# wzf2000/GAMER

Measured on AMD Instinct MI355X. Metric: train-step sequences/sec, Qwen3Multi SMB decoder, his_len=100, higher is better.
Workload: dtype f32 tensors/accumulators, products = 3 x fp16 pieces (split3)

## Files before the change

### gamer_amd/_lib.py

```python
from __future__ import annotations

import ctypes as C
import os
import re
from typing import Optional

import torch

_HERE = os.path.dirname(os.path.abspath(__file__))
LIB_PATH = os.path.join(_HERE, "lib", "libgamer_hip.so")
if os.environ.get("GAMER_LIB_PATH"):
    LIB_PATH = os.path.abspath(os.environ["GAMER_LIB_PATH"])
HEADER_PATH = os.path.join(os.path.dirname(_HERE), "include", "gamer_hip.h")

_lib: Optional[C.CDLL] = None

c_void_p, c_int, c_float, c_int64, c_uint64 = C.c_void_p, C.c_int, C.c_float, C.c_int64, C.c_uint64


class GemmDesc(C.Structure):
    _fields_ = [
        ("A", c_void_p), ("a_rs", c_int64), ("a_ks", c_int64),
        ("B", c_void_p), ("b_rs", c_int64), ("b_ks", c_int64),
        ("C", c_void_p), ("ldc", c_int64),
        ("M", c_int), ("N", c_int), ("K", c_int),
        ("alpha", c_float),
        ("accumulate", c_int),
        ("groups", c_int),
        ("group_mode", c_int),
        ("group_offsets", c_void_p),
        ("strideB", c_int64), ("strideC", c_int64),
        ("kchunk", c_int),
        ("resid", c_void_p),
        ("row_map", c_void_p),
        ("p_drop", c_float),
        ("seed", c_uint64),
        ("rowdot_other", c_void_p),
        ("rowdot_out", c_void_p),
        ("rowdot_S", c_int),
        ("qk_wq", c_void_p), ("qk_wk", c_void_p),
        ("qk_eps", c_float),
        ("qk_cos", c_void_p), ("qk_sin", c_void_p),
        ("qk_bias_q", c_void_p), ("qk_bias_k", c_void_p), ("qk_bias_v", c_void_p),
        ("qk_act_idx", c_void_p),
        ("qk_pos_ids", c_void_p),
        ("qk_q_rot", c_void_p), ("qk_k_rot", c_void_p),
        ("qk_S", c_int), ("qk_nq", c_int), ("qk_nkv", c_int),
        ("b_planes", c_void_p), ("b_plane_stride", c_int64),
        ("amax_a", c_void_p), ("amax_b", c_void_p),
        ("amax_c", c_void_p), ("amax_c_col0", c_int),
        ("wgrad_ws", c_void_p), ("wgrad_ws_floats", c_int64),
        ("sw_gu", c_void_p), ("sw_ld", c_int64),
        ("group_div", c_int), ("sw_tbl", c_void_p), ("b_planes_t", c_void_p),
        ("sw_hm", c_void_p), ("sw_row_group", c_void_p),
    ]


class GemmBf16Desc(C.Structure):
    _fields_ = [
        ("A", c_void_p), ("lda", c_int64),
        ("B", c_void_p), ("ldb", c_int64),
        ("C", c_void_p), ("ldc", c_int64),
        ("M", c_int), ("N", c_int), ("K", c_int),
        ("accumulate", c_int),
        ("groups", c_int),
        ("group_mode", c_int),
        ("group_offsets", c_void_p),
        ("strideB", c_int64), ("strideC", c_int64),
        ("kchunk", c_int),
        ("resid", c_void_p),
        ("row_map", c_void_p),
        ("p_drop", c_float),
        ("seed", c_uint64),
        ("rowdot_other", c_void_p),
        ("rowdot_out", c_void_p),
        ("rowdot_S", c_int),
        ("qk_wq", c_void_p), ("qk_wk", c_void_p), ("qk_eps", c_float),
        ("qk_cos", c_void_p), ("qk_sin", c_void_p),
        ("qk_bias_q", c_void_p), ("qk_bias_k", c_void_p), ("qk_bias_v", c_void_p),
        ("qk_act_idx", c_void_p), ("qk_pos_ids", c_void_p),
        ("qk_q_rot", c_void_p), ("qk_k_rot", c_void_p),
        ("qk_S", c_int), ("qk_nq", c_int), ("qk_nkv", c_int),
        ("sw_gu", c_void_p), ("sw_ld", c_int64),
        ("wgrad_ws", c_void_p), ("wgrad_ws_floats", c_int64),
    ]


P, I, F, L, U = c_void_p, c_int, c_float, c_int64, c_uint64

_SIGNATURES = {
    "gamer_router_fwd": [P, P, P, P, I, I, I, I, I, I, P, P, P, P, P, P, P, P, P, P, P, P],
    "gamer_expert_lists": [P, I, I, I, P, P, P, P, P],
    "gamer_causal_prep": [P, I, I, P, P, P, P, P, P],
    "gamer_session_prep": [P, P, P, I, I, I, I, P, P, P, P, P, P, P],
    "gamer_moe_router_prep": [P, P, P, I, P, I, I, I, I, I, I, I, P, P, P, P, P, P, P, P, P],
    "gamer_embedding_fwd": [P, P, I, I, I, P, P],
    "gamer_embedding_bwd": [P, P, I, I, I, I, P, P],
    "gamer_embedding_bwd_ordered": [P, P, I, I, I, I, P, P, L, P],
    "gamer_embedding_bwd_ordered_ws_bytes": [I, I, I],
    "gamer_rmsnorm_fwd": [P, P, I, I, F, P, P, I, P],
    "gamer_rmsnorm_bwd": [P, P, P, I, P, I, I, F, I, P, P, I, P, P, F, U, P],
    "gamer_colsum_reduce": [P, I, I, I, P, P],
    "gamer_colsum_reduce_batched": [P, L, I, I, I, P, I, P],
    "gamer_rowtable_fwd": [P, P, P, I, I, P, I, I, P],
    "gamer_rowtable_bwd": [P, I, I, P, P, I, I, I, P, P, L, P],
    "gamer_gemm_f32": [C.POINTER(GemmDesc), P],
    "gamer_gemm_f32_split": [C.POINTER(GemmDesc), c_int, P],
    "gamer_split3_guard": [I],
    "gamer_gemm_bf16": [C.POINTER(GemmBf16Desc), P],
    "gamer_cast_params_bf16": [P, P, P, P, I, I, P],
    "gamer_attn_fwd_bf16": [P, I, P, I, P, I, P, P, I, I, I, I, F, F, U, P, P, P, P, P, P, P],
    "gamer_attn_bwd_bf16": [P, I, P, I, P, I, P, P, P, P, P, I, I, I, I, F, F, U, P, P, I, P, I, P, I, P, I, P, P, P, P],
    "gamer_session_spans": [P, P, P, P, P, I, I, I, I, P, P, P, P, P, P, P, P, P],
    "gamer_qknorm_rope_fwd": [P, I, I, I, I, P, P, F, P, P, P, P, P, P, P, P, P, P],
    "gamer_qknorm_rope_bwd": [P, P, P, I, I, I, I, P, P, F, P, P, P, P, P, I, P, P, P, P, P, P, P, P, L, P],
    "gamer_attn_row_order": [P, I, I, P, P, P, P],
    "gamer_attn_fwd": [P, I, P, I, P, I, P, P, P, P, I, I, I, I, F, F, U, P, P, P, P, P, I, P, P],
    "gamer_attn_bwd": [P, I, P, I, P, I, P, P, P, P, P, P, P, I, I, I, I, F, F, U, P, P, I, P, I, P, I, P, P, P, P, P, I, P],
    "gamer_split3_planes": [P, P, L, L, P],
    "gamer_absmax_f32": [P, I, L, I, I, L, P, P],
    "gamer_absmax_multi_f32": [P, P, I, P, P],
    "gamer_split2h_planes_multi": [P, P, I, P, P, P],
    "gamer_amax_sink": [P, P],
    "gamer_amax_sink3": [P, P, P],
    "gamer_attn_split_amax": [P, P, P, P],
    "gamer_attn_fwd_split": [P, I, P, I, P, I, P, P, P, I, I, I, I, F, F, U, P, P, P, P, P, I, P, P],
    "gamer_attn_bwd_split": [P, I, P, I, P, I, P, P, P, P, P, P, P, I, I, I, I, F, F, U, P, P, I, P, I, P, I, P, P, P, I, P, P, P],
    "gamer_residual_dropout_fwd": [P, P, P, I, I, F, U, P, P],
    "gamer_residual_dropout_bwd": [P, P, I, I, F, U, P, P],
    "gamer_swiglu_fwd": [P, P, L, F, U, P, P],
    "gamer_swiglu_bwd": [P, P, P, L, F, U, P],
    "gamer_swiglu_fwd_ld": [P, L, I, I, F, U, P, P],
    "gamer_swiglu_bwd_ld": [P, L, I, I, P, F, U, P],
    "gamer_swiglu_fwd_ld_tbl": [P, L, I, I, F, U, P, P, P, P],
    "gamer_swiglu_bwd_ld_tbl": [P, L, I, I, P, F, U, P, P, P],
    "gamer_silu_fwd_ld": [P, L, I, I, F, U, P, P],
    "gamer_silu_bwd_ld": [P, L, I, I, P, F, U, P],
# ... 113 lines not shown
```

### gamer_amd/csrc/common.h

```cpp
#pragma once
#include <hip/hip_runtime.h>
#include <stdint.h>
#include <stdio.h>
#include <stdarg.h>
#include <stdlib.h>

#include "../../include/gamer_hip.h"

namespace gamer {

void set_error(const char* fmt, ...);

#define GAMER_CHECK_ARG(cond, ...)                       \
    do {                                                 \
        if (!(cond)) {                                   \
            gamer::set_error(__VA_ARGS__);               \
            return -1;                                   \
        }                                                \
    } while (0)

#define GAMER_CHECK_LAUNCH(name)                                                        \
    do {                                                                                \
        hipError_t e__ = hipGetLastError();                                             \
        if (e__ != hipSuccess) {                                                        \
// ... 161 lines not shown
    __device__ __forceinline__ float mult(uint64_t idx) const {
        if (!on) return 1.f;
        uint32_t h = mix32((uint32_t)idx ^ k0);
        h = mix32(h + (uint32_t)(idx >> 32) * 0x9e3779b1U + k1);
        return h >= thr ? scale : 0.f;
    }
};

struct AttnDropout {
    uint32_t k0, k1, thr;
    float scale;
    __device__ __forceinline__ AttnDropout(float p, uint64_t seed) {
        k0 = mix32((uint32_t)seed ^ 0x9e3779b9U) ^ mix32((uint32_t)(seed >> 32) + 0x7f4a7c15U);
        k1 = mix32(k0 + 0x632be5abU);
        const float t = p * 4294967296.f;
        thr = t >= 4294967040.f ? 0xffffffffU : (uint32_t)t;
        scale = p > 0.f ? 1.f / (1.f - p) : 1.f;
    }
    __device__ __forceinline__ uint32_t row_word(uint32_t row) const {
        return (mix32(row * 0x9e3779b1U + k0) & 0xffffffU) | 0x800001U;
    }
    __device__ __forceinline__ uint32_t key_word(uint32_t j) const { return mix32(j * 0x85ebca6bU + k1) & 0xffffffU; }
    __device__ __forceinline__ bool keep(uint32_t a, uint32_t b) const { return __umul24(a, b) >= thr; }
};

__device__ __forceinline__ float xor32_max(float v) {
    const auto sw = __builtin_amdgcn_permlane32_swap(__float_as_uint(v), __float_as_uint(v), false, false);
    return fmaxf(__uint_as_float(sw[0]), __uint_as_float(sw[1]));
}
__device__ __forceinline__ float xor32_sum(float v) {
    const auto sw = __builtin_amdgcn_permlane32_swap(__float_as_uint(v), __float_as_uint(v), false, false);
    return __uint_as_float(sw[0]) + __uint_as_float(sw[1]);
}

__device__ __forceinline__ int wave_sum_i32(int v) {
#pragma unroll
    for (int o = 32; o > 0; o >>= 1) v += __shfl_xor(v, o, 64);
    return v;
}
__device__ __forceinline__ int wave_max_i32(int v) {
#pragma unroll
    for (int o = 32; o > 0; o >>= 1) v = max(v, __shfl_xor(v, o, 64));
    return v;
}
__device__ __forceinline__ int wave_min_i32(int v) {
#pragma unroll
    for (int o = 32; o > 0; o >>= 1) v = min(v, __shfl_xor(v, o, 64));
    return v;
}

#define GAMER_DPP_ROW_REDUCE(OP, v)                                                                   \
    v = OP(v, __builtin_amdgcn_update_dpp(v, v, 0xB1, 0xf, 0xf, false));      \
    v = OP(v, __builtin_amdgcn_update_dpp(v, v, 0x4E, 0xf, 0xf, false));      \
    v = OP(v, __builtin_amdgcn_update_dpp(v, v, 0x141, 0xf, 0xf, false));         \
    v = OP(v, __builtin_amdgcn_update_dpp(v, v, 0x140, 0xf, 0xf, false));
__device__ __forceinline__ int wave_min_i32_dpp(int v) {
    GAMER_DPP_ROW_REDUCE(min, v)
    return min(min(__builtin_amdgcn_readlane(v, 0), __builtin_amdgcn_readlane(v, 16)),
               min(__builtin_amdgcn_readlane(v, 32), __builtin_amdgcn_readlane(v, 48)));
}
__device__ __forceinline__ int wave_max_i32_dpp(int v) {
    GAMER_DPP_ROW_REDUCE(max, v)
    return max(max(__builtin_amdgcn_readlane(v, 0), __builtin_amdgcn_readlane(v, 16)),
               max(__builtin_amdgcn_readlane(v, 32), __builtin_amdgcn_readlane(v, 48)));
}

__device__ __forceinline__ float row16_sum_dpp(float v) {
#define GAMER_DPP_F(ctrl) __int_as_float(__builtin_amdgcn_update_dpp(__float_as_int(v), __float_as_int(v), ctrl, 0xf, 0xf, false))
    v += GAMER_DPP_F(0xB1);
    v += GAMER_DPP_F(0x4E);
    v += GAMER_DPP_F(0x141);
    v += GAMER_DPP_F(0x140);
#undef GAMER_DPP_F
    return v;
}

__device__ __forceinline__ float sigmoid_f(float x) { return __builtin_amdgcn_rcpf(1.f + __expf(-x)); }
__device__ __forceinline__ float silu_f(float x) { return x * sigmoid_f(x); }
__device__ __forceinline__ float dsilu_f(float x) {
    const float s = sigmoid_f(x);
    return s * (1.f + x * (1.f - s));
}

bool gemm_as_eligible(const gamer_gemm_desc* d, bool a_kc, bool b_kc, const uint16_t* b_planes);
int launch_gemm_as(const gamer_gemm_desc* d, const uint16_t* b_planes, bool b_kc, hipStream_t st);
bool gemm_os_eligible(const gamer_gemm_desc* d, bool a_kc, bool b_kc, const uint16_t* b_planes);
int launch_gemm_os(const gamer_gemm_desc* d, const uint16_t* b_planes, int guard, hipStream_t st, bool fwd_t = false);
bool gemm_os_fwd_eligible(const gamer_gemm_desc* d, bool a_kc, bool b_kc);
bool gemm_wg_eligible(const gamer_gemm_desc* d, bool a_kc, bool b_kc);
int launch_gemm_wg(const gamer_gemm_desc* d, hipStream_t st);

int launch_wgrad_reduce(const float* ws, float* C, int64_t ldc, int M, int N, int groups, const int32_t* group_offsets, int K,
                        int kchunk, int64_t strideC, hipStream_t st);

}
```

### gamer_amd/csrc/elementwise.hip

```cpp
#include "common.h"

namespace gamer {

constexpr int EW_THREADS = 256;
constexpr int EW_WAVES = EW_THREADS / WAVE;

#ifndef EW_MAX_BLOCKS_W
#define EW_MAX_BLOCKS_W 8192
#endif
#ifndef EW_MAX_BLOCKS_T
#define EW_MAX_BLOCKS_T 16384
#endif
static inline int grid_for_waves(int64_t n_waves, int max_blocks = EW_MAX_BLOCKS_W) {
    int64_t blocks = (n_waves + EW_WAVES - 1) / EW_WAVES;
    if (blocks < 1) blocks = 1;
    if (blocks > max_blocks) blocks = max_blocks;
    return (int)blocks;
}
static inline int grid_for_threads(int64_t n, int max_blocks = EW_MAX_BLOCKS_T) {
    int64_t blocks = (n + EW_THREADS - 1) / EW_THREADS;
    if (blocks < 1) blocks = 1;
    if (blocks > max_blocks) blocks = max_blocks;
    return (int)blocks;
}
// ... 149 lines not shown
            int rank = 0, cnt = 0;
            for (int j = 0; j < 64; ++j) {
                const int bj = __shfl(b, j, 64);
                const bool same = bj == b;
                rank += (same && j < lane) ? 1 : 0;
                cnt += same ? 1 : 0;
            }
            if (b >= 0) {
                const int pos = emb_cur[b] + rank;
                perm[pos] = t;
                __builtin_amdgcn_wave_barrier();
                if (rank == cnt - 1) emb_cur[b] = pos + 1;
            }
            __builtin_amdgcn_wave_barrier();
        }
    }
}

__global__ void __launch_bounds__(EW_THREADS)
emb_piece_sum_kernel(const float4* __restrict__ dx, int V, int H4, const int* __restrict__ row_start, const int* __restrict__ row_count,
                     const int* __restrict__ piece_start, const int* __restrict__ perm, float4* __restrict__ partial) {
    __shared__ float4 red[3][256];
    const int p = blockIdx.x;
    if (p >= piece_start[V]) return;
    int lo = 0, hi = V;
    while (hi - lo > 1) { const int mid = (lo + hi) >> 1; if (piece_start[mid] <= p) lo = mid; else hi = mid; }
    const int v = lo, k = p - piece_start[v];
    const int begin = row_start[v] + k * EMB_PIECE;
    const int count = min(EMB_PIECE, row_count[v] - k * EMB_PIECE);
    const int lane = threadIdx.x & 63, w = threadIdx.x >> 6;
    for (int c0 = 0; c0 < H4; c0 += 64) {
        const int c = c0 + lane;
        float4 acc = make_float4(0.f, 0.f, 0.f, 0.f);
        if (c < H4) {
            const int j1 = min(count, (w + 1) * (EMB_PIECE / 4));
            int j = w * (EMB_PIECE / 4);
            for (; j + 4 <= j1; j += 4) {
                const int r0 = perm[begin + j], r1 = perm[begin + j + 1], r2 = perm[begin + j + 2], r3 = perm[begin + j + 3];
                const float4 a0 = dx[(int64_t)r0 * H4 + c], a1 = dx[(int64_t)r1 * H4 + c], a2 = dx[(int64_t)r2 * H4 + c],
                             a3 = dx[(int64_t)r3 * H4 + c];
                acc.x = (((acc.x + a0.x) + a1.x) + a2.x) + a3.x; acc.y = (((acc.y + a0.y) + a1.y) + a2.y) + a3.y;
                acc.z = (((acc.z + a0.z) + a1.z) + a2.z) + a3.z; acc.w = (((acc.w + a0.w) + a1.w) + a2.w) + a3.w;
            }
            for (; j < j1; ++j) {
                const float4 a0 = dx[(int64_t)perm[begin + j] * H4 + c];
                acc.x += a0.x; acc.y += a0.y; acc.z += a0.z; acc.w += a0.w;
            }
        }
        if (w > 0 && c < H4) red[w - 1][lane] = acc;
        __syncthreads();
        if (w == 0 && c < H4) {
            const float4 b = red[0][lane], d = red[1][lane], e = red[2][lane];
            float4 o;
            o.x = (acc.x + b.x) + (d.x + e.x); o.y = (acc.y + b.y) + (d.y + e.y);
            o.z = (acc.z + b.z) + (d.z + e.z); o.w = (acc.w + b.w) + (d.w + e.w);
            partial[(int64_t)p * H4 + c] = o;
        }
        __syncthreads();
    }
}

__global__ void __launch_bounds__(64)
emb_row_sum_kernel(int H4, const int* __restrict__ piece_start, const float4* __restrict__ partial, float4* __restrict__ dW) {
    const int v = blockIdx.x;
    const int p0 = piece_start[v], p1 = piece_start[v + 1];
    if (p0 == p1) return;
    for (int c = threadIdx.x; c < H4; c += 64) {
        float4 s = partial[(int64_t)p0 * H4 + c];
        for (int p = p0 + 1; p < p1; ++p) {
            const float4 a = partial[(int64_t)p * H4 + c];
            s.x += a.x; s.y += a.y; s.z += a.z; s.w += a.w;
        }
        float4 o = dW[(int64_t)v * H4 + c];
        o.x += s.x; o.y += s.y; o.z += s.z; o.w += s.w;
        dW[(int64_t)v * H4 + c] = o;
    }
}

constexpr int RMS_MAXC_BIG = 4;

template <typename TY, int RMS_MAXC>
__global__ void __launch_bounds__(EW_THREADS)
rmsnorm_fwd_kernel(const float4* __restrict__ x, const float4* __restrict__ w, int T, int H4, float inv_h,
                   float eps, const int32_t* __restrict__ dst_rows, TY* __restrict__ y, int ldy, uint32_t* __restrict__ amax_out) {
    __shared__ uint32_t amax_lds[4];
    uint32_t am = 0;
    const int lane = threadIdx.x & 63;
    const int wave = (blockIdx.x * EW_THREADS + threadIdx.x) >> 6;
    const int nwaves = (gridDim.x * EW_THREADS) >> 6;
    float4 wv[RMS_MAXC];
#pragma unroll
    for (int i = 0; i < RMS_MAXC; ++i) {
        const int c = lane + 64 * i;
        wv[i] = (c < H4) ? w[c] : make_float4(0.f, 0.f, 0.f, 0.f);
    }
    for (int t = wave; t < T; t += nwaves) {
        float4 v[RMS_MAXC];
        float ss = 0.f;
#pragma unroll
        for (int i = 0; i < RMS_MAXC; ++i) {
            const int c = lane + 64 * i;
            v[i] = (c < H4) ? x[(int64_t)t * H4 + c] : make_float4(0.f, 0.f, 0.f, 0.f);
            ss += v[i].x * v[i].x + v[i].y * v[i].y + v[i].z * v[i].z + v[i].w * v[i].w;
        }
        ss = wave_sum(ss);
        const float rstd = rsqrtf(ss * inv_h + eps);
        const int64_t r = dst_rows ? dst_rows[t] : t;
        TY* yrow = y + r * ldy;
#pragma unroll
        for (int i = 0; i < RMS_MAXC; ++i) {
            const int c = lane + 64 * i;
            if (c < H4) {
                float4 o;
                o.x = wv[i].x * (v[i].x * rstd);
                o.y = wv[i].y * (v[i].y * rstd);
                o.z = wv[i].z * (v[i].z * rstd);
                o.w = wv[i].w * (v[i].w * rstd);
                st4(yrow + 4 * c, o);
                am = amax_f4(am, o);
            }
        }
    }
    amax_block_commit(am, amax_out, amax_lds);
}

template <typename TG, int RMS_MAXC>
__global__ void __launch_bounds__(EW_THREADS)
rmsnorm_bwd_kernel(const float4* __restrict__ x, const float4* __restrict__ w, const TG* __restrict__ dy,
                   int lddy, const int32_t* __restrict__ dy_rows, int T, int H4, float inv_h, float eps,
                   int accumulate_dx, float4* __restrict__ dx, float* __restrict__ dw_partial,
                   TG* __restrict__ mask_out, const int32_t* __restrict__ mask_rows, float p_drop, uint64_t seed,
                   uint32_t* __restrict__ amax_out) {
    const DropoutRng rng(mask_out ? p_drop : 0.f, seed);
    __shared__ float4 red[EW_WAVES][64 * RMS_MAXC];
    __shared__ uint32_t amax_lds[4];
    uint32_t am = 0;
    const int lane = threadIdx.x & 63;
    const int wib = threadIdx.x >> 6;
    const int wave = (blockIdx.x * EW_THREADS + threadIdx.x) >> 6;
    const int nwaves = (gridDim.x * EW_THREADS) >> 6;
    float4 wv[RMS_MAXC], dwacc[RMS_MAXC];
#pragma unroll
    for (int i = 0; i < RMS_MAXC; ++i) {
        const int c = lane + 64 * i;
        wv[i] = (c < H4) ? w[c] : make_float4(0.f, 0.f, 0.f, 0.f);
        dwacc[i] = make_float4(0.f, 0.f, 0.f, 0.f);
    }
    for (int t = wave; t < T; t += nwaves) {
        float4 v[RMS_MAXC], g[RMS_MAXC];
        float ss = 0.f;
        const int64_t r = dy_rows ? dy_rows[t] : t;
        const TG* dyrow = dy + r * lddy;
#pragma unroll
        for (int i = 0; i < RMS_MAXC; ++i) {
            const int c = lane + 64 * i;
            v[i] = (c < H4) ? x[(int64_t)t * H4 + c] : make_float4(0.f, 0.f, 0.f, 0.f);
            g[i] = (c < H4) ? ld4(dyrow + 4 * c) : make_float4(0.f, 0.f, 0.f, 0.f);
            ss += v[i].x * v[i].x + v[i].y * v[i].y + v[i].z * v[i].z + v[i].w * v[i].w;
        }
        ss = wave_sum(ss);
        const float rstd = rsqrtf(ss * inv_h + eps);
        float dot = 0.f;
#pragma unroll
        for (int i = 0; i < RMS_MAXC; ++i) {
            v[i].x *= rstd; v[i].y *= rstd; v[i].z *= rstd; v[i].w *= rstd;
            dwacc[i].x += g[i].x * v[i].x; dwacc[i].y += g[i].y * v[i].y;
            dwacc[i].z += g[i].z * v[i].z; dwacc[i].w += g[i].w * v[i].w;
            g[i].x *= wv[i].x; g[i].y *= wv[i].y; g[i].z *= wv[i].z; g[i].w *= wv[i].w;
            dot += g[i].x * v[i].x + g[i].y * v[i].y + g[i].z * v[i].z + g[i].w * v[i].w;
        }
        dot = wave_sum(dot) * inv_h;
#pragma unroll
        for (int i = 0; i < RMS_MAXC; ++i) {
            const int c = lane + 64 * i;
            if (c < H4) {
                float4 o;
                o.x = rstd * (g[i].x - v[i].x * dot);
                o.y = rstd * (g[i].y - v[i].y * dot);
                o.z = rstd * (g[i].z - v[i].z * dot);
                o.w = rstd * (g[i].w - v[i].w * dot);
                if (accumulate_dx) {
                    float4 p = dx[(int64_t)t * H4 + c];
                    o.x += p.x; o.y += p.y; o.z += p.z; o.w += p.w;
                }
                dx[(int64_t)t * H4 + c] = o;
                if (mask_out) {
                    float m[4];
                    rng.mult4((uint32_t)((int64_t)t * H4 + c), m);
                    const int64_t mr = mask_rows ? mask_rows[t] : t;
                    const float4 mo = make_float4(m[0] * o.x, m[1] * o.y, m[2] * o.z, m[3] * o.w);
                    st4(mask_out + (mr * H4 + c) * 4, mo);
                    am = amax_f4(am, mo);
                }
            }
        }
    }
#pragma unroll
    for (int i = 0; i < RMS_MAXC; ++i) red[wib][lane + 64 * i] = dwacc[i];
    __syncthreads();
    if (wib == 0) {
// ... 1366 lines not shown
extern "C" int gamer_amax_sink(uint32_t* out0, uint32_t* out1) {
    g_amax_sink.out[0] = out0;
    g_amax_sink.out[1] = out1;
    g_amax_sink.out[2] = nullptr;
    return 0;
}
extern "C" int gamer_amax_sink3(uint32_t* out0, uint32_t* out1, uint32_t* out2) {
    g_amax_sink.out[0] = out0;
    g_amax_sink.out[1] = out1;
    g_amax_sink.out[2] = out2;
    return 0;
}

extern "C" int gamer_embedding_fwd(const int64_t* ids, const float* W, int V, int T, int H, float* x, void* stream) {
    GAMER_CHECK_ARG(ids && W && x, "gamer_embedding_fwd: null pointer");
    GAMER_CHECK_ARG(T > 0 && H > 0 && H % 4 == 0 && V > 0, "gamer_embedding_fwd: bad shape T=%d H=%d V=%d", T, H, V);
    GAMER_CHECK_ARG(aligned16(W) && aligned16(x), "gamer_embedding_fwd: pointers must be 16-byte aligned");
    hipLaunchKernelGGL(embedding_fwd_kernel, dim3(grid_for_waves(T)), dim3(EW_THREADS), 0, ST(stream),
                       ids, (const float4*)W, V, T, H / 4, (float4*)x);
    GAMER_CHECK_LAUNCH("gamer_embedding_fwd");
    return 0;
}

extern "C" int gamer_embedding_bwd(const int64_t* ids, const float* dx, int V, int T, int H, int pad_id, float* dW,
                                   void* stream) {
    GAMER_CHECK_ARG(ids && dx && dW, "gamer_embedding_bwd: null pointer");
    GAMER_CHECK_ARG(T > 0 && H > 0 && V > 0, "gamer_embedding_bwd: bad shape T=%d H=%d V=%d", T, H, V);
    GAMER_CHECK_ARG(H <= 1024, "gamer_embedding_bwd: H=%d > 1024 unsupported", H);
    int chunk = EMB_CHUNK;
    while (chunk > 128 && (T + chunk - 1) / chunk < 512) chunk >>= 1;
    hipLaunchKernelGGL(embedding_bwd_kernel, dim3((T + chunk - 1) / chunk), dim3(EW_THREADS),
                       (size_t)EMB_CACHE * H * sizeof(float), ST(stream), ids, dx, V, T, H, pad_id, dW, chunk);
    GAMER_CHECK_LAUNCH("gamer_embedding_bwd");
    return 0;
}

extern "C" int64_t gamer_embedding_bwd_ordered_ws_bytes(int V, int T, int H) {
    if (V <= 0 || T <= 0 || H <= 0) return -1;
    const int64_t chunks = (T + EMB_SORT_CHUNK - 1) / EMB_SORT_CHUNK;
    const int64_t pieces = (int64_t)T / EMB_PIECE + V + 1;
    const int64_t ints = chunks * (V + 1) + 2 * (int64_t)(V + 1) + (V + 2) + T;
    return ((ints * 4 + 15) / 16) * 16 + pieces * H * 4;
}
extern "C" int gamer_embedding_bwd_ordered(const int64_t* ids, const float* dx, int V, int T, int H, int pad_id, float* dW,
                                           void* ws, int64_t ws_bytes, void* stream) {
    GAMER_CHECK_ARG(ids && dx && dW && ws, "gamer_embedding_bwd_ordered: null pointer");
    GAMER_CHECK_ARG(T > 0 && H > 0 && H % 4 == 0 && V > 0 && V <= EMB_MAX_V,
                    "gamer_embedding_bwd_ordered: bad shape T=%d H=%d V=%d (H %% 4 == 0, V <= %d)", T, H, V, EMB_MAX_V);
    GAMER_CHECK_ARG(aligned16(dx) && aligned16(dW) && aligned16(ws) && ws_bytes >= gamer_embedding_bwd_ordered_ws_bytes(V, T, H),
                    "gamer_embedding_bwd_ordered: dx / dW / ws must be 16-byte aligned and ws hold %lld bytes (got %lld)",
                    (long long)gamer_embedding_bwd_ordered_ws_bytes(V, T, H), (long long)ws_bytes);
    const int chunks = (T + EMB_SORT_CHUNK - 1) / EMB_SORT_CHUNK;
    const int pieces_max = T / EMB_PIECE + V + 1;
    int* ip = (int*)ws;
    EmbSortWs w;
    w.hist = ip; ip += (int64_t)chunks * (V + 1);
    w.row_start = ip; ip += V + 1;
    w.row_count = ip; ip += V + 1;
    w.piece_start = ip; ip += V + 2;
    w.perm = ip; ip += T;
    const int64_t ints = (int64_t)chunks * (V + 1) + 2 * (int64_t)(V + 1) + (V + 2) + T;
    w.partial = (float*)((char*)ws + ((ints * 4 + 15) / 16) * 16);
    hipStream_t st = ST(stream);
    const size_t lds = (size_t)(V + 1) * sizeof(int);
    hipLaunchKernelGGL(emb_hist_kernel, dim3(chunks), dim3(EW_THREADS), lds, st, ids, V, T, pad_id, w.hist);
    GAMER_CHECK_LAUNCH("gamer_embedding_bwd_ordered/hist");
    hipLaunchKernelGGL(emb_chunk_scan_kernel, dim3(V + 1), dim3(64), 0, st, V, chunks, w.hist, w.row_count);
    GAMER_CHECK_LAUNCH("gamer_embedding_bwd_ordered/chunk_scan");
    hipLaunchKernelGGL(emb_row_scan_kernel, dim3(1), dim3(1024), 0, st, V, w.row_count, w.row_start, w.piece_start);
    GAMER_CHECK_LAUNCH("gamer_embedding_bwd_ordered/row_scan");
    hipLaunchKernelGGL(emb_scatter_kernel, dim3(chunks), dim3(EW_THREADS), lds + EMB_SORT_CHUNK * sizeof(int), st, ids, V, T, pad_id,
                       w.hist, w.row_start, w.perm);
    GAMER_CHECK_LAUNCH("gamer_embedding_bwd_ordered/scatter");
    hipLaunchKernelGGL(emb_piece_sum_kernel, dim3(pieces_max), dim3(EW_THREADS), 0, st, (const float4*)dx, V, H / 4, w.row_start,
                       w.row_count, w.piece_start, w.perm, (float4*)w.partial);
    GAMER_CHECK_LAUNCH("gamer_embedding_bwd_ordered/pieces");
    hipLaunchKernelGGL(emb_row_sum_kernel, dim3(V), dim3(64), 0, st, H / 4, w.piece_start, (const float4*)w.partial, (float4*)dW);
    GAMER_CHECK_LAUNCH("gamer_embedding_bwd_ordered/rows");
    return 0;
}

template <typename TY>
static int rmsnorm_fwd_impl(const char* name, const float* x, const float* w, int T, int H, float eps,
                            const int32_t* dst_rows, TY* y, int ldy, void* stream) {
    GAMER_CHECK_ARG(x && w && y, "%s: null pointer", name);
    GAMER_CHECK_ARG(T > 0 && H > 0 && H % 4 == 0 && H <= 256 * RMS_MAXC_BIG && ldy >= H && ldy % 4 == 0,
                    "%s: bad shape T=%d H=%d ldy=%d (H%%4==0, H<=1024, ldy%%4==0)", name, T, H, ldy);
    GAMER_CHECK_ARG(aligned16(x) && aligned16(w) && aligned_vec4<TY>(y), "%s: pointers must be 16-byte aligned", name);
    const AmaxSink sink = take_amax_sink();
    if (H <= 256)
        hipLaunchKernelGGL((rmsnorm_fwd_kernel<TY, 1>), dim3(grid_for_waves(T)), dim3(EW_THREADS), 0, ST(stream),
                           (const float4*)x, (const float4*)w, T, H / 4, 1.f / (float)H, eps, dst_rows, y, ldy, sink.out[0]);
    else
        hipLaunchKernelGGL((rmsnorm_fwd_kernel<TY, RMS_MAXC_BIG>), dim3(grid_for_waves(T)), dim3(EW_THREADS), 0, ST(stream),
                           (const float4*)x, (const float4*)w, T, H / 4, 1.f / (float)H, eps, dst_rows, y, ldy, sink.out[0]);
    GAMER_CHECK_LAUNCH(name);
    return 0;
}
extern "C" int gamer_rmsnorm_fwd(const float* x, const float* w, int T, int H, float eps, const int32_t* dst_rows,
                                 float* y, int ldy, void* stream) {
    return rmsnorm_fwd_impl<float>("gamer_rmsnorm_fwd", x, w, T, H, eps, dst_rows, y, ldy, stream);
}
extern "C" int gamer_rmsnorm_fwd_bf16(const float* x, const float* w, int T, int H, float eps, const int32_t* dst_rows,
                                      gamer_bf16* y, int ldy, void* stream) {
    return rmsnorm_fwd_impl<bf16_t>("gamer_rmsnorm_fwd_bf16", x, w, T, H, eps, dst_rows, (bf16_t*)y, ldy, stream);
}

template <typename TG>
static int rmsnorm_bwd_impl(const char* name, const float* x, const float* w, const TG* dy, int lddy,
                            const int32_t* dy_rows, int T, int H, float eps, int accumulate_dx, float* dx,
                            float* dw_partial, int n_partial, TG* mask_out, const int32_t* mask_rows, float p_drop,
                            uint64_t seed, void* stream) {
    GAMER_CHECK_ARG(x && w && dy && dx && dw_partial, "%s: null pointer", name);
    GAMER_CHECK_ARG(T > 0 && H > 0 && H % 4 == 0 && H <= 256 * RMS_MAXC_BIG && lddy >= H && lddy % 4 == 0 && n_partial > 0,
                    "%s: bad shape T=%d H=%d lddy=%d n_partial=%d", name, T, H, lddy, n_partial);
    GAMER_CHECK_ARG(aligned16(x) && aligned16(w) && aligned_vec4<TG>(dy) && aligned16(dx) && aligned16(dw_partial) &&
                    aligned_vec4<TG>(mask_out), "%s: pointers must be 16-byte aligned", name);
    const AmaxSink sink = take_amax_sink();
    if (H <= 256)
        hipLaunchKernelGGL((rmsnorm_bwd_kernel<TG, 1>), dim3(n_partial), dim3(EW_THREADS), 0, ST(stream),
                           (const float4*)x, (const float4*)w, dy, lddy, dy_rows, T, H / 4, 1.f / (float)H, eps,
                           accumulate_dx, (float4*)dx, dw_partial, mask_out, mask_rows, p_drop, seed, sink.out[0]);
    else
        hipLaunchKernelGGL((rmsnorm_bwd_kernel<TG, RMS_MAXC_BIG>), dim3(n_partial), dim3(EW_THREADS), 0, ST(stream),
                           (const float4*)x, (const float4*)w, dy, lddy, dy_rows, T, H / 4, 1.f / (float)H, eps,
                           accumulate_dx, (float4*)dx, dw_partial, mask_out, mask_rows, p_drop, seed, sink.out[0]);
    GAMER_CHECK_LAUNCH(name);
    return 0;
}
extern "C" int gamer_rmsnorm_bwd(const float* x, const float* w, const float* dy, int lddy, const int32_t* dy_rows,
                                 int T, int H, float eps, int accumulate_dx, float* dx, float* dw_partial,
                                 int n_partial, float* mask_out, const int32_t* mask_rows, float p_drop,
                                 uint64_t seed, void* stream) {
    return rmsnorm_bwd_impl<float>("gamer_rmsnorm_bwd", x, w, dy, lddy, dy_rows, T, H, eps, accumulate_dx, dx, dw_partial,
                                   n_partial, mask_out, mask_rows, p_drop, seed, stream);
}
extern "C" int gamer_rmsnorm_bwd_bf16(const float* x, const float* w, const gamer_bf16* dy, int lddy,
                                      const int32_t* dy_rows, int T, int H, float eps, int accumulate_dx, float* dx,
                                      float* dw_partial, int n_partial, gamer_bf16* mask_out, const int32_t* mask_rows,
                                      float p_drop, uint64_t seed, void* stream) {
    return rmsnorm_bwd_impl<bf16_t>("gamer_rmsnorm_bwd_bf16", x, w, (const bf16_t*)dy, lddy, dy_rows, T, H, eps,
                                    accumulate_dx, dx, dw_partial, n_partial, (bf16_t*)mask_out, mask_rows, p_drop, seed,
                                    stream);
}

extern "C" int gamer_colsum_reduce(const float* partial, int rows, int cols, int accumulate, float* out, void* stream) {
    GAMER_CHECK_ARG(partial && out && rows > 0 && cols > 0, "gamer_colsum_reduce: bad arguments");
    hipLaunchKernelGGL(colsum_reduce_kernel, dim3((cols + 31) / 32), dim3(32 * COLSUM_RG), 0, ST(stream), partial, rows,
                       cols, accumulate, out);
    GAMER_CHECK_LAUNCH("gamer_colsum_reduce");
    return 0;
}

extern "C" int gamer_colsum_reduce_batched(const float* partial, int64_t stride, int rows, int cols, int n, float* const* outs,
                                           int accumulate, void* stream) {
    GAMER_CHECK_ARG(partial && outs && rows > 0 && cols > 0 && n > 0 && n <= 65535 && stride >= (int64_t)rows * cols,
                    "gamer_colsum_reduce_batched: bad arguments (rows=%d cols=%d n=%d stride=%lld)", rows, cols, n, (long long)stride);
    hipLaunchKernelGGL(colsum_reduce_batched_kernel, dim3((cols + 31) / 32, n), dim3(32 * COLSUM_RG), 0, ST(stream), partial, stride,
                       rows, cols, accumulate, outs);
    GAMER_CHECK_LAUNCH("gamer_colsum_reduce_batched");
    return 0;
}

template <typename TY>
static int rowtable_fwd_impl(const char* name, const float* table, const int32_t* idx, const int32_t* dst_rows, int T,
                             int E, TY* y, int ldy, int col0, void* stream) {
    GAMER_CHECK_ARG(table && idx && y, "%s: null pointer", name);
    GAMER_CHECK_ARG(T > 0 && E > 0 && E % 4 == 0 && ldy % 4 == 0 && col0 % 4 == 0 && col0 + E <= ldy,
                    "%s: bad shape T=%d E=%d ldy=%d col0=%d", name, T, E, ldy, col0);
    hipLaunchKernelGGL(rowtable_fwd_kernel<TY>, dim3(grid_for_threads((int64_t)T * E / 4)), dim3(EW_THREADS), 0,
                       ST(stream), (const float4*)table, idx, dst_rows, T, E / 4, y, ldy, col0, take_amax_sink().out[0]);
    GAMER_CHECK_LAUNCH(name);
    return 0;
}
extern "C" int gamer_rowtable_fwd(const float* table, const int32_t* idx, const int32_t* dst_rows, int T, int E,
                                  float* y, int ldy, int col0, void* stream) {
    return rowtable_fwd_impl<float>("gamer_rowtable_fwd", table, idx, dst_rows, T, E, y, ldy, col0, stream);
}
extern "C" int gamer_rowtable_fwd_bf16(const float* table, const int32_t* idx, const int32_t* dst_rows, int T, int E,
                                       gamer_bf16* y, int ldy, int col0, void* stream) {
    return rowtable_fwd_impl<bf16_t>("gamer_rowtable_fwd_bf16", table, idx, dst_rows, T, E, (bf16_t*)y, ldy, col0, stream);
}

template <typename TG>
// ... 496 lines not shown
```

### gamer_amd/csrc/gemm.hip

```cpp
#include "common.h"
#include <stdlib.h>

namespace gamer {

constexpr int BM = 128, BN = 128, BK = 32;
constexpr int GEMM_THREADS = 256;
constexpr int KC_LD = BK + 4;
constexpr int TILE_FLOATS = BM * KC_LD;
constexpr int GEMM_LDS_BYTES = 4 * TILE_FLOATS * (int)sizeof(float);

typedef float f32x16 __attribute__((ext_vector_type(16)));

constexpr int SP_KC_ROW = 80;
constexpr int SP_KC_IMG = BM * SP_KC_ROW;
constexpr int SP_RC_IMG = BK * 256;
constexpr int SP_OPERAND = 3 * SP_KC_IMG;
constexpr int SP_LDS_BYTES = 2 * SP_OPERAND;

#ifndef SP_ABLATE
#define SP_ABLATE 0
#endif
__device__ __forceinline__ uint32_t pack_hi16(uint32_t w0, uint32_t w1) { return __builtin_amdgcn_perm(w1, w0, 0x07060302u); }
__device__ __forceinline__ void split3(float x, uint32_t (&w)[3]) {
    if (SP_ABLATE & 1) { w[0] = w[1] = w[2] = __float_as_uint(x); return; }
// ... 1295 lines not shown
static int gemm_entry(const gamer_gemm_desc* d, void* stream, int split) {
    GAMER_CHECK_ARG(d, "gamer_gemm_f32: null descriptor");
    GAMER_CHECK_ARG(d->A && d->B && d->C, "gamer_gemm_f32: null matrix pointer");
    GAMER_CHECK_ARG(d->M > 0 && d->N > 0 && d->K > 0, "gamer_gemm_f32: bad shape M=%d N=%d K=%d", d->M, d->N, d->K);
    GAMER_CHECK_ARG((d->a_rs == 1) != (d->a_ks == 1) || (d->a_rs == 1 && d->a_ks == 1 && (d->M == 1 || d->K == 1)),
                    "gamer_gemm_f32: exactly one of a_rs/a_ks must be 1 (rs=%lld ks=%lld)", (long long)d->a_rs, (long long)d->a_ks);
    GAMER_CHECK_ARG((d->b_rs == 1) != (d->b_ks == 1) || (d->b_rs == 1 && d->b_ks == 1 && (d->N == 1 || d->K == 1)),
                    "gamer_gemm_f32: exactly one of b_rs/b_ks must be 1 (rs=%lld ks=%lld)", (long long)d->b_rs, (long long)d->b_ks);
    const bool a_kc = d->a_ks == 1, b_kc = d->b_ks == 1;
    const int64_t a_ld = a_kc ? d->a_rs : d->a_ks, b_ld = b_kc ? d->b_rs : d->b_ks;
    GAMER_CHECK_ARG(a_ld % 4 == 0 && b_ld % 4 == 0 && d->ldc >= d->N,
                    "gamer_gemm_f32: leading dims must be multiples of 4 (lda=%lld ldb=%lld ldc=%lld)",
                    (long long)a_ld, (long long)b_ld, (long long)d->ldc);
    GAMER_CHECK_ARG(aligned16(d->A) && aligned16(d->B), "gamer_gemm_f32: A and B must be 16-byte aligned");
    GAMER_CHECK_ARG(d->groups >= 1 && (d->groups == 1 || d->group_offsets), "gamer_gemm_f32: groups=%d needs group_offsets", d->groups);
    GAMER_CHECK_ARG(d->strideB % 4 == 0, "gamer_gemm_f32: strideB must be a multiple of 4");
    GAMER_CHECK_ARG(d->group_mode == 0 || d->group_mode == 1, "gamer_gemm_f32: group_mode=%d", d->group_mode);

    GemmParams p;
    p.A = d->A; p.a_rs = d->a_rs; p.a_ks = d->a_ks;
    p.B = d->B; p.b_rs = d->b_rs; p.b_ks = d->b_ks;
    p.C = d->C; p.ldc = d->ldc;
    p.M = d->M; p.N = d->N; p.K = d->K;
    p.alpha = d->alpha; p.accumulate = d->accumulate;
    p.groups = d->groups; p.group_offsets = d->group_offsets;
    p.strideB = d->strideB; p.strideC = d->strideC;
    p.kchunk = d->kchunk;
    p.resid = d->resid; p.row_map = d->row_map; p.p_drop = d->p_drop; p.seed = d->seed;
    p.rowdot_other = d->rowdot_other; p.rowdot_out = d->rowdot_out; p.rowdot_S = d->rowdot_S;
    p.qk_wq = d->qk_wq; p.qk_wk = d->qk_wk; p.qk_eps = d->qk_eps; p.qk_cos = d->qk_cos; p.qk_sin = d->qk_sin;
    p.qk_bias_q = d->qk_bias_q; p.qk_bias_k = d->qk_bias_k; p.qk_bias_v = d->qk_bias_v;
    p.qk_act_idx = d->qk_act_idx; p.qk_pos_ids = d->qk_pos_ids; p.qk_q_rot = d->qk_q_rot; p.qk_k_rot = d->qk_k_rot;
    p.qk_S = d->qk_S; p.qk_nq = d->qk_nq; p.qk_nkv = d->qk_nkv;
    p.amax_a = d->amax_a; p.amax_b = d->amax_b;
    p.guard = g_split3_guard;
    p.amax_c = d->amax_c; p.amax_c_col0 = d->amax_c_col0;
    p.wgrad_ws = nullptr;
    p.sw_gu = d->sw_gu; p.sw_ld = d->sw_ld;
    p.group_div = d->group_div > 1 ? d->group_div : 1; p.sw_tbl = d->sw_tbl;
    GAMER_CHECK_ARG(d->group_div <= 1 || (d->group_mode == 0 && d->group_offsets && d->groups % d->group_div == 0),
                    "gamer_gemm_f32: group_div = %d needs group_mode 0, group_offsets and groups (%d) a multiple of it", d->group_div, d->groups);
    GAMER_CHECK_ARG(!d->sw_tbl || ((d->sw_gu || d->sw_hm) && aligned16(d->sw_tbl)),
                    "gamer_gemm_f32: sw_tbl is an option of the SwiGLU epilogues (sw_gu, sw_hm)");
    GAMER_CHECK_ARG(!d->sw_gu || (split == 3 && d->group_mode == 0 && !d->accumulate && !d->resid && !d->rowdot_out && !d->qk_q_rot &&
                                  d->alpha == 1.f && d->N % 4 == 0 && d->sw_ld >= 2 * (int64_t)d->N && d->sw_ld % 4 == 0 &&
                                  aligned16(d->sw_gu) && d->p_drop >= 0.f && d->p_drop < 1.f),
                    "gamer_gemm_f32: the SwiGLU-backward epilogue (sw_gu) is built for gamer_gemm_f32_split(terms = 3), a plain input-"
                    "gradient GEMM with alpha = 1, N %% 4 == 0, sw_ld >= 2 N (N=%d sw_ld=%lld)", d->N, (long long)d->sw_ld);
    GAMER_CHECK_ARG(!d->amax_c || (d->group_mode == 0 && !d->accumulate && !d->resid && !d->qk_q_rot && d->amax_c_col0 >= 0 &&
                                   d->amax_c_col0 % 64 == 0),
                    "gamer_gemm_f32: amax_c needs a plain or row-dot Linear-forward / input-gradient GEMM (no accumulate, residual or "
                    "q|k|v epilogue) and amax_c_col0 a multiple of 64 (amax_c_col0=%d)", d->amax_c_col0);
    GAMER_CHECK_ARG(split != 3 || (d->amax_a && d->amax_b), "gamer_gemm_f32_split: terms = 3 needs amax_a and amax_b (gamer_absmax_f32)");
    p.b_planes = (split && d->group_mode == 0) ? (const uint16_t*)d->b_planes : nullptr;
    p.b_plane_stride = d->b_plane_stride;
    GAMER_CHECK_ARG(!p.b_planes || split == 3 || ((reinterpret_cast<uintptr_t>(p.b_planes) & 7u) == 0 && d->b_plane_stride % 4 == 0 && d->b_plane_stride > 0),
                    "gamer_gemm_f32_split: b_planes must be 8-byte aligned with b_plane_stride %% 4 == 0");
    GAMER_CHECK_ARG(!p.b_planes || split != 3 || (reinterpret_cast<uintptr_t>(p.b_planes) & 15u) == 0,
                    "gamer_gemm_f32_split: terms = 3 takes b_planes as packed pieces at B's offsets (16-byte aligned)");
    if (split == 3 && p.b_planes && ((b_kc ? d->K : d->N) % 4) != 0) p.b_planes = nullptr;
    GAMER_CHECK_ARG(!d->qk_q_rot || (d->qk_k_rot && d->qk_wq && d->qk_wk && d->qk_cos && d->qk_sin && d->group_mode == 0 &&
                                     d->groups == 1 && a_kc && b_kc && !d->resid && !d->rowdot_out && !d->accumulate &&
                                     d->alpha == 1.f && d->M % BM == 0 && d->qk_nq > 0 && d->qk_nkv > 0 && d->qk_S > 0 &&
                                     d->N == (d->qk_nq + 2 * d->qk_nkv) * 64 && d->N % BN == 0 && d->ldc % 4 == 0 &&
                                     aligned16(d->C) && aligned16(d->qk_q_rot) && aligned16(d->qk_k_rot) &&
                                     (!d->qk_bias_q || (d->qk_bias_k && d->qk_bias_v && d->qk_act_idx)) &&
                                     !diag_build_switches()),
                    "gamer_gemm_f32: the q|k|v epilogue needs a Linear-forward layout, one group, M %% 128 == 0 (M=%d), "
                    "N = (nq + 2 nkv) * 64 a multiple of 128 (N=%d), alpha = 1 and no other epilogue", d->M, d->N);
    GAMER_CHECK_ARG(!d->rowdot_out || (d->rowdot_other && d->rowdot_S > 0 && d->group_mode == 0 && d->groups == 1 &&
                                       !d->resid && !d->accumulate && d->M % BM == 0 && d->N % BN == 0 &&
                                       d->M % d->rowdot_S == 0 && d->ldc % 4 == 0 && aligned16(d->rowdot_other) &&
                                       aligned16(d->C) && !diag_build_switches()),
                    "gamer_gemm_f32: the row-dot epilogue needs full 128 x 128 tiles (M=%d N=%d), one group, ldc %% 4 == 0",
                    d->M, d->N);
    GAMER_CHECK_ARG(!d->resid || (d->group_mode == 0 && !d->accumulate && a_kc && b_kc && d->ldc % 4 == 0 &&
                                  aligned16(d->resid) && aligned16(d->C) && d->p_drop >= 0.f && d->p_drop < 1.f),
                    "gamer_gemm_f32: the fused residual epilogue needs a Linear-forward layout, ldc %% 4 == 0, no accumulate");
    GAMER_CHECK_ARG(!d->sw_hm || (d->group_mode == 0 && a_kc && b_kc && !d->accumulate && !d->resid && !d->rowdot_out && !d->qk_q_rot &&
                                  !d->sw_gu && d->alpha == 1.f && d->N % 8 == 0 && d->ldc >= d->N && d->ldc % 4 == 0 && aligned16(d->sw_hm) &&
                                  aligned16(d->C) && (!d->sw_tbl || d->sw_row_group) && d->p_drop >= 0.f && d->p_drop < 1.f),
                    "gamer_gemm_f32: the SwiGLU-forward epilogue (sw_hm) needs a Linear-forward layout with N = 2 I (N=%d), alpha = 1, no other "
                    "epilogue, and sw_row_group with sw_tbl", d->N);
    if (split == 3 && gemm_as_eligible(d, a_kc, b_kc, p.b_planes)) return launch_gemm_as(d, p.b_planes, b_kc, (hipStream_t)stream);
    if (d->sw_hm) {
        gamer_gemm_desc d2 = *d;
        d2.sw_hm = nullptr; d2.sw_row_group = nullptr; d2.sw_tbl = nullptr; d2.amax_c = nullptr;
        const int rc = gemm_entry(&d2, stream, split);
        if (rc) return rc;
        if (d->amax_c) gamer_amax_sink(d->amax_c, nullptr);
        return d->sw_tbl ? gamer_swiglu_fwd_ld_tbl(d->C, d->ldc, d->M, d->N / 2, d->p_drop, d->seed, d->sw_hm, d->sw_tbl, d->sw_row_group, stream)
                         : gamer_swiglu_fwd_ld(d->C, d->ldc, d->M, d->N / 2, d->p_drop, d->seed, d->sw_hm, stream);
    }
    if (split == 3 && gemm_os_eligible(d, a_kc, b_kc, p.b_planes)) return launch_gemm_os(d, p.b_planes, g_split3_guard, (hipStream_t)stream);
    if (split == 3 && gemm_os_fwd_eligible(d, a_kc, b_kc))
        return launch_gemm_os(d, reinterpret_cast<const uint16_t*>(d->b_planes_t), g_split3_guard, (hipStream_t)stream, true);
    p.n_tiles = (d->N + BN - 1) / BN;
    hipStream_t st = (hipStream_t)stream;

    if (d->group_mode == 0) {
        p.m_tiles = (d->M + BM - 1) / BM + (d->group_offsets ? d->groups : 0);
        const int64_t blocks = (int64_t)p.m_tiles * p.n_tiles;
        GAMER_CHECK_ARG(blocks < (1LL << 31), "gamer_gemm_f32: grid too large");
        if (a_kc && b_kc) return launch_gemm<true, true, 0>(p, (int)blocks, st, split);
        if (a_kc && !b_kc) return launch_gemm<true, false, 0>(p, (int)blocks, st, split);
        if (!a_kc && !b_kc) return launch_gemm<false, false, 0>(p, (int)blocks, st, split);
        GAMER_CHECK_ARG(false, "gamer_gemm_f32: layout (A row-contiguous, B k-contiguous) is not built");
    } else {
        GAMER_CHECK_ARG(!a_kc && !b_kc, "gamer_gemm_f32: group_mode 1 (wgrad) needs row-contiguous A and B");
        GAMER_CHECK_ARG(d->kchunk >= BK && d->kchunk % BK == 0, "gamer_gemm_f32: kchunk=%d must be a positive multiple of 32", d->kchunk);
        p.m_tiles = (d->M + BM - 1) / BM;
        const int64_t chunks = (d->K + d->kchunk - 1) / d->kchunk + (d->group_offsets ? d->groups : 0);
        const int64_t blocks = chunks * p.m_tiles * p.n_tiles;
        GAMER_CHECK_ARG(blocks < (1LL << 31), "gamer_gemm_f32: grid too large");
        p.wgrad_ws = d->wgrad_ws;
        if (p.wgrad_ws) {
            const int64_t need = chunks * p.m_tiles * p.n_tiles * (int64_t)(BM * BN);
            GAMER_CHECK_ARG(d->wgrad_ws_floats >= need && aligned16(d->wgrad_ws),
                            "gamer_gemm_f32: wgrad_ws holds %lld floats, this weight gradient needs %lld (chunks x tiles x 16384)",
                            (long long)d->wgrad_ws_floats, (long long)need);
            GAMER_CHECK_ARG(!diag_pp_switch(), "gamer_gemm_f32: the deterministic weight gradient is not built for the ping-pong form");
        }
        const int rc = (split == 3 && p.wgrad_ws && gemm_wg_eligible(d, a_kc, b_kc)) ? launch_gemm_wg(d, st)
                                                                                     : launch_gemm<false, false, 1>(p, (int)blocks, st, split);
        if (rc || !p.wgrad_ws) return rc;
        const int64_t rblocks = (int64_t)d->groups * p.m_tiles * p.n_tiles * 16;
        hipLaunchKernelGGL(wgrad_reduce_kernel, dim3((int)rblocks), dim3(256), 0, st, p.wgrad_ws, d->C, d->ldc, d->M, d->N, p.m_tiles,
                           p.n_tiles, d->groups, d->group_offsets, d->K, d->kchunk, d->strideC);
        GAMER_CHECK_LAUNCH("gamer_gemm_f32/wgrad_reduce");
        return 0;
    }
    return 0;
}

__device__ __forceinline__ uint32_t amax4(uint32_t m, const uint4 v) {
    return max(max(m, v.x & 0x7fffffffu), max(max(v.y & 0x7fffffffu, v.z & 0x7fffffffu), v.w & 0x7fffffffu));
}
__device__ __forceinline__ void amax_commit(uint32_t m, uint32_t* __restrict__ out) {
    __shared__ uint32_t part[4];
#pragma unroll
    for (int o = 32; o > 0; o >>= 1) m = max(m, (uint32_t)__shfl_xor((int)m, o, 64));
    if ((threadIdx.x & 63) == 0) part[threadIdx.x >> 6] = m;
    __syncthreads();
    if (threadIdx.x == 0) {
        m = max(max(part[0], part[1]), max(part[2], part[3]));
        if (m) amax_publish(m, out, blockIdx.x);
    }
}
__global__ void __launch_bounds__(256)
absmax_flat_kernel(const uint4* __restrict__ x, int64_t n4, uint32_t* __restrict__ out) {
    uint32_t m = 0;
    const int64_t step = (int64_t)gridDim.x * 256;
    int64_t i = (int64_t)blockIdx.x * 256 + threadIdx.x;
    for (; i + step < n4; i += 2 * step) {
        const uint4 a = x[i], b = x[i + step];
        m = amax4(amax4(m, a), b);
    }
    if (i < n4) m = amax4(m, x[i]);
    amax_commit(m, out);
}
__global__ void __launch_bounds__(256)
absmax_rows_kernel(const float* __restrict__ x, int batch, int64_t stride, int rows, int cols, int64_t ld, uint32_t* __restrict__ out) {
    const int lane = threadIdx.x & 63;
    const int64_t waves = (int64_t)gridDim.x * 4, nrows = (int64_t)batch * rows;
    uint32_t m = 0;
    for (int64_t w = (int64_t)blockIdx.x * 4 + (threadIdx.x >> 6); w < nrows; w += waves) {
        const int64_t b = w / rows, r = w - b * rows;
// ... 120 lines not shown
```

### gamer_amd/csrc/gemm_as.hip

```cpp
#include "common.h"
#include <stdlib.h>
#include <atomic>

namespace gamer {

typedef float f32x16 __attribute__((ext_vector_type(16)));
typedef uint32_t u32x4a __attribute__((ext_vector_type(4)));

#ifndef AS_WAVES
#define AS_WAVES 4
#endif
#ifndef AS_NT
#define AS_NT 1
#endif
#ifndef AS_DEPTH
#define AS_DEPTH 1
#endif
#ifndef AS_ABLATE
#define AS_ABLATE 0
#endif
constexpr int AS_SLAB = 32 * AS_NT;
constexpr int AS_PANEL = AS_SLAB * 64;

__device__ __forceinline__ int as_f(int row) { return (((row >> 1) & 1) << 2) | (((row >> 3) & 1) << 1) | ((row >> 2) & 1); }
__device__ __forceinline__ int as_off(int row, int col) { return row * 64 + ((((col >> 3) ^ as_f(row))) << 3) + (col & 7); }

struct AsParams {
    const float* A; int64_t lda;
    const uint16_t* Wp;
    int64_t ldw;
    float* C; int64_t ldc;
    int M, N, K;
    float alpha;
    const uint32_t* amax_w;
    uint32_t* amax_c; int amax_c_col0;
    int groups; const int32_t* group_offsets; int64_t strideW;
    int accumulate;
    const float* rowdot_other; float* rowdot_out; int rowdot_S;
    float* sw_gu; int64_t sw_ld; float p_drop; uint64_t seed;
    float* hm; const float* tbl; int group_div;
};

template <int KP, bool WRC, int EPI, int NW>
__global__ void __launch_bounds__(64 * NW, AS_DEPTH == 2 ? 1 : 8 / NW)
gemm_as_kernel(const AsParams p) {
    constexpr int AS_WAVES_K = NW, AS_THREADS_K = 64 * NW;
    extern __shared__ __attribute__((aligned(16))) unsigned char as_raw[];
    bf16_t* const wimg = reinterpret_cast<bf16_t*>(as_raw);
    __shared__ uint32_t amax_word;
    const int tid = threadIdx.x, lane = tid & 63, w = tid >> 6;
    const int r = lane & 31, h = lane >> 5;
    int row0 = blockIdx.x * (32 * AS_WAVES_K), row_end = p.M, grp = 0;
    if (p.group_offsets) {
        int prev = p.group_offsets[0], tiles_before = 0;
        bool found = false;
        for (int gi = 0; gi < p.groups; ++gi) {
            const int nxt = p.group_offsets[gi + 1];
            const int tiles = (nxt - prev + 32 * AS_WAVES_K - 1) / (32 * AS_WAVES_K);
            if (!found && (int)blockIdx.x < tiles_before + tiles) {
                grp = gi; row0 = prev + ((int)blockIdx.x - tiles_before) * (32 * AS_WAVES_K); row_end = nxt; found = true;
            }
            if (!found) tiles_before += tiles;
            prev = nxt;
        }
        if (!found) return;
    }
    const int m = row0 + w * 32 + r;
    const bool valid_m = m < row_end;
    if (tid == 0) amax_word = 0;

    bf16x8 af[2][KP * 4];
    float row_inv;
    {
        const float* arow = p.A + (int64_t)(valid_m ? m : row_end - 1) * p.lda + 8 * h;
        float4 raw[KP * 8];
#pragma unroll
        for (int s = 0; s < KP * 4; ++s) {
            raw[2 * s] = *reinterpret_cast<const float4*>(arow + 16 * s);
            raw[2 * s + 1] = *reinterpret_cast<const float4*>(arow + 16 * s + 4);
        }
        float mx = 0.f;
#pragma unroll
        for (int i = 0; i < KP * 8; ++i) {
            if (!valid_m) raw[i] = make_float4(0.f, 0.f, 0.f, 0.f);
            mx = fmaxf(fmaxf(fmaxf(mx, fabsf(raw[i].x)), fabsf(raw[i].y)), fmaxf(fabsf(raw[i].z), fabsf(raw[i].w)));
        }
        mx = xor32_max(mx);
        float s_row = 1.f;
        row_inv = 1.f;
        if (mx > 0.f) scale_from_amax(__float_as_uint(mx), s_row, row_inv);
#pragma unroll
        for (int s = 0; s < KP * 4; ++s) {
            u32x4a u0, u1;
#pragma unroll
            for (int j = 0; j < 2; ++j) {
                const float4 x = raw[2 * s + j];
                uint32_t a0, a1, b0, b1;
                cut2h_quad(x.x, x.y, x.z, x.w, s_row, a0, a1, b0, b1);
                u0[2 * j] = a0; u0[2 * j + 1] = b0; u1[2 * j] = a1; u1[2 * j + 1] = b1;
            }
            af[0][s] = __builtin_bit_cast(bf16x8, u0);
            af[1][s] = __builtin_bit_cast(bf16x8, u1);
        }
    }
    float w_s, w_inv;
    scale_from_amax(amax_read(p.amax_w), w_s, w_inv);
    const float out_scale = row_inv * w_inv * p.alpha;

    const int n_slabs = (p.N + AS_SLAB - 1) / AS_SLAB;
    constexpr int QPR = KP * 16;
    constexpr int NLD = AS_SLAB * QPR / AS_THREADS_K;
    uint4 rw[NLD], rw2[NLD];
    int lds_off[NLD], nl_[NLD];
    const uint4* wsrc[NLD];
#pragma unroll
    for (int i = 0; i < NLD; ++i) {
        const int f = tid + AS_THREADS_K * i;
        if (!WRC) {
            const int nl = f / QPR, g = f % QPR;
            nl_[i] = nl;
            lds_off[i] = (g >> 4) * AS_PANEL + as_off(nl, (4 * g) & 63);
            wsrc[i] = reinterpret_cast<const uint4*>(p.Wp) + (((int64_t)(grp / p.group_div) * p.strideW + (int64_t)nl * p.ldw + 4 * g) >> 2);
        } else {
            const int k = f / (AS_SLAB / 4), nq = f % (AS_SLAB / 4);
            nl_[i] = 4 * nq;
            lds_off[i] = k * AS_SLAB + 4 * nq;
            wsrc[i] = reinterpret_cast<const uint4*>(p.Wp) + (((int64_t)(grp / p.group_div) * p.strideW + (int64_t)k * p.ldw + 4 * nq) >> 2);
        }
    }
    const int64_t slab_stride = WRC ? (AS_SLAB >> 2) : (((int64_t)AS_SLAB * p.ldw) >> 2);
    auto load_slab_into = [&](int j, uint4 (&dst)[NLD]) {
        const bool full = (j + 1) * AS_SLAB <= p.N;
#pragma unroll
        for (int i = 0; i < NLD; ++i) {
            const uint4* src = wsrc[i] + (int64_t)j * slab_stride;
            if (!full && j * AS_SLAB + nl_[i] >= p.N) src = wsrc[i];
            dst[i] = *src;
        }
    };
    auto store_slab_from = [&](int j, int buf, const uint4 (&rw)[NLD]) {
        bf16_t* img = wimg + buf * (2 * KP * AS_PANEL);
        const bool full = (j + 1) * AS_SLAB <= p.N;
#pragma unroll
        for (int i = 0; i < NLD; ++i) {
            const bool ok = full || j * AS_SLAB + nl_[i] < p.N;
            *reinterpret_cast<uint2*>(img + lds_off[i]) = ok ? make_uint2(rw[i].x, rw[i].y) : make_uint2(0u, 0u);
            *reinterpret_cast<uint2*>(img + KP * AS_PANEL + lds_off[i]) = ok ? make_uint2(rw[i].z, rw[i].w) : make_uint2(0u, 0u);
        }
    };
    auto load_slab = [&](int j) { load_slab_into(j, rw); };
    auto store_slab = [&](int j, int buf) { store_slab_from(j, buf, rw); };
    int row_off[4];
#pragma unroll
    for (int s = 0; s < 4; ++s) row_off[s] = as_off(r, 16 * s + 8 * h);
    const int tr_lane = (8 * h + ((lane >> 2) & 3)) * AS_SLAB + 16 * ((lane >> 4) & 1) + 4 * (lane & 3);
    auto read_tr = [&](const bf16_t* base) -> bf16x8 {
        bf16x8 out;
#pragma unroll
        for (int c = 0; c < 2; ++c) {
            const bf16x4 v = __builtin_amdgcn_ds_read_tr16_b64_v4bf16((bf16x4 __attribute__((address_space(3)))*)(base + c * 4 * AS_SLAB));
            out[4 * c + 0] = v[0]; out[4 * c + 1] = v[1]; out[4 * c + 2] = v[2]; out[4 * c + 3] = v[3];
        }
        return out;
    };
    float hd_dot = 0.f;
    float emax = 0.f;
    float4 gsave[EPI == 5 ? 4 * AS_NT : 1];
    float* const tbl_lds = reinterpret_cast<float*>(as_raw + (size_t)(AS_DEPTH == 2 ? 3 : 2) * 2 * KP * AS_PANEL * sizeof(bf16_t));
    if (EPI == 5 && p.tbl) {
        const float4* src = reinterpret_cast<const float4*>(p.tbl + (int64_t)grp * p.N);
// ... 65 lines not shown
                            if (col + 4 <= p.N) {
                                *reinterpret_cast<float4*>(crow + col) = t4;
                            } else {
                                const float e[4] = {t4.x, t4.y, t4.z, t4.w};
                                for (int q = 0; q < 4 && col + q < p.N; ++q) crow[col + q] = e[q];
                            }
                            if (EPI == 2) {
                                const float4 o4 = *reinterpret_cast<const float4*>(p.rowdot_other + (int64_t)m * p.ldc + col);
                                part += (t4.x * o4.x + t4.y * o4.y) + (t4.z * o4.z + t4.w * o4.w);
                            }
                            if (EPI == 5) {
                                const int half = p.N >> 1;
                                float4 x4 = t4;
                                if (p.tbl) {
                                    const float4 tb = *reinterpret_cast<const float4*>(tbl_lds + col);
                                    x4.x += tb.x; x4.y += tb.y; x4.z += tb.z; x4.w += tb.w;
                                }
                                if (col < half) {
                                    gsave[EPI == 5 ? nt * 4 + g4 : 0] = x4;
                                } else {
                                    const float4 g = gsave[EPI == 5 ? nt * 4 + g4 : 0];
                                    const int hc = col - half;
                                    const DropoutRng rng(p.p_drop, p.seed);
                                    float mu[4];
                                    rng.mult4((uint32_t)(((int64_t)m * half + hc) >> 2), mu);
                                    const float4 o = make_float4(mu[0] * (silu_f(g.x) * x4.x), mu[1] * (silu_f(g.y) * x4.y),
                                                                 mu[2] * (silu_f(g.z) * x4.z), mu[3] * (silu_f(g.w) * x4.w));
                                    *reinterpret_cast<float4*>(p.hm + (int64_t)m * half + hc) = o;
                                    emax = fmaxf(fmaxf(fmaxf(emax, fabsf(o.x)), fabsf(o.y)), fmaxf(fabsf(o.z), fabsf(o.w)));
                                }
                            }
                            if (track) cmax = fmaxf(fmaxf(fmaxf(cmax, fabsf(t4.x)), fabsf(t4.y)), fmaxf(fabsf(t4.z), fabsf(t4.w)));
                        }
                    }
            }
            if (EPI == 2) {
                const float sl = xor32_sum(part);
                constexpr int SPH = 64 / AS_SLAB;
                hd_dot = (j % SPH == 0) ? sl : hd_dot + sl;
                if (j % SPH == SPH - 1 && valid_m && h == 0) {
                    const int heads = p.N >> 6, head = (j * AS_SLAB) >> 6;
                    p.rowdot_out[((int64_t)(m / p.rowdot_S) * heads + head) * p.rowdot_S + m % p.rowdot_S] = hd_dot;
                }
            }
    };
    if (AS_DEPTH == 1) {
        load_slab(0);
        store_slab(0, 0);
        __syncthreads();
        auto slab_of = [&](int i) { return EPI == 5 ? (i >> 1) + (i & 1) * (n_slabs >> 1) : i; };
#pragma unroll 1
        for (int i = 0; i < n_slabs; ++i) {
            const int j = slab_of(i), buf = i & 1, jn = slab_of(min(i + 1, n_slabs - 1));
            if (!(AS_ABLATE & 4)) load_slab(jn);
            __builtin_amdgcn_sched_barrier(0);
            mfma_slab(j, buf);
            __builtin_amdgcn_sched_barrier(0);
            if (!(AS_ABLATE & 4)) store_slab(jn, buf ^ 1);
            epilogue_slab(j);
            __syncthreads();
        }
    } else {
        load_slab_into(0, rw);
        store_slab_from(0, 0, rw);
        if (n_slabs > 1) load_slab_into(1, rw);
        if (n_slabs > 2) load_slab_into(2, rw2);
        __syncthreads();
        int bufc = 0;
#pragma unroll 1
        for (int j = 0; j < n_slabs; j += 2) {
            const int b1 = bufc == 2 ? 0 : bufc + 1, b2 = b1 == 2 ? 0 : b1 + 1;
            mfma_slab(j, bufc); epilogue_slab(j);
            if (j + 1 < n_slabs) store_slab_from(j + 1, b1, rw);
            if (j + 3 < n_slabs) load_slab_into(j + 3, rw);
            __syncthreads();
            if (j + 1 >= n_slabs) break;
            mfma_slab(j + 1, b1); epilogue_slab(j + 1);
            if (j + 2 < n_slabs) store_slab_from(j + 2, b2, rw2);
            if (j + 4 < n_slabs) load_slab_into(j + 4, rw2);
            __syncthreads();
            bufc = b2;
        }
    }
    if (p.amax_c) {
        uint32_t mw = __float_as_uint((EPI == 4 || EPI == 5) ? emax : cmax);
#pragma unroll
        for (int o2 = 32; o2 > 0; o2 >>= 1) mw = max(mw, (uint32_t)__shfl_xor((int)mw, o2, 64));
        if (lane == 0 && mw) atomicMax(&amax_word, mw);
        __syncthreads();
        if (tid == 0 && amax_word) amax_publish(amax_word, p.amax_c, blockIdx.x);
    }
}

static std::atomic<long long> g_as_launches{0};

static inline bool gemm_as_enabled() {
    static EnvSwitch sw("GAMER_GEMM_AS");
    return sw.get(1) != 0;
}

bool gemm_as_eligible(const gamer_gemm_desc* d, bool a_kc, bool b_kc, const uint16_t* b_planes) {
    if (!gemm_as_enabled() || !a_kc || !b_planes || !d->amax_b) return false;
    if (d->group_mode != 0 || d->resid || d->qk_q_rot) return false;
    if ((d->group_div > 1 || d->sw_tbl) && !d->sw_hm) return false;
    if (d->sw_hm) {
        static EnvSwitch sw5("GAMER_GEMM_AS_SWIGLU");
        if (sw5.get(1) == 0 || !b_kc || d->accumulate || d->rowdot_out || d->sw_gu || d->N % (2 * AS_SLAB) != 0 || d->alpha != 1.f ||
            !aligned16(d->sw_hm) || (d->sw_tbl && (!aligned16(d->sw_tbl) || !d->group_offsets)) || d->p_drop < 0.f || d->p_drop >= 1.f)
            return false;
        if (d->group_div > 1 && (!d->group_offsets || d->groups % d->group_div != 0)) return false;
    }
    static EnvSwitch min_m("GAMER_GEMM_AS_MIN_M");
    if (d->K % 64 != 0 || d->K < 64 || d->K > 256 || d->M < min_m.get(16384)) return false;
    if (d->a_rs % 4 != 0 || d->ldc % 4 != 0 || !aligned16(d->C) || !aligned16(b_planes)) return false;
    if (d->groups != 1 && (!d->group_offsets || d->strideC != 0)) return false;
    if (d->groups == 1 && d->group_offsets) return false;
    if (b_kc) {
        if (d->accumulate || d->rowdot_out || d->sw_gu || d->b_rs % 4 != 0) return false;
        if (d->groups != 1 && d->amax_c && !d->sw_hm) return false;
        if (d->amax_c && !d->sw_hm && d->amax_c_col0 % AS_SLAB != 0) return false;
        return true;
    }
    static EnvSwitch rc("GAMER_GEMM_AS_RC");
    const int rc_mode = rc.get(1);
    if (rc_mode == 0) return false;
    if (d->K != 256 || d->N % 4 != 0 || d->b_ks % 4 != 0) return false;
    if ((d->sw_gu || d->rowdot_out) && rc_mode < 2) return false;
    if (d->sw_gu) {
        return !d->amax_c || d->amax_c_col0 == 0;
    }
    if (d->groups != 1) return false;
    if (d->rowdot_out) return !d->accumulate && d->N % 64 == 0 && 64 % AS_SLAB == 0 && (!d->amax_c || d->amax_c_col0 % AS_SLAB == 0);
    return !d->amax_c || (!d->accumulate && d->amax_c_col0 % AS_SLAB == 0);
}

int launch_gemm_as(const gamer_gemm_desc* d, const uint16_t* b_planes, bool b_kc, hipStream_t st) {
    AsParams p;
    p.A = d->A; p.lda = d->a_rs;
    p.Wp = b_planes; p.ldw = b_kc ? d->b_rs : d->b_ks;
    p.C = d->C; p.ldc = d->ldc;
    p.M = d->M; p.N = d->N; p.K = d->K;
    p.alpha = d->alpha;
    p.amax_w = d->amax_b;
    p.amax_c = d->amax_c; p.amax_c_col0 = d->amax_c_col0;
    p.groups = d->groups; p.group_offsets = d->groups > 1 ? d->group_offsets : nullptr; p.strideW = d->strideB;
    p.accumulate = d->accumulate;
    p.rowdot_other = d->rowdot_other; p.rowdot_out = d->rowdot_out; p.rowdot_S = d->rowdot_S;
    p.sw_gu = d->sw_gu; p.sw_ld = d->sw_ld; p.p_drop = d->p_drop; p.seed = d->seed;
    p.hm = d->sw_hm; p.tbl = d->sw_hm ? d->sw_tbl : nullptr; p.group_div = d->group_div > 1 ? d->group_div : 1;
    const int kp = d->K / 64;
    const size_t shmem = (size_t)(AS_DEPTH == 2 ? 3 : 2) * 2 * kp * AS_PANEL * sizeof(bf16_t) + (d->sw_hm ? (size_t)d->N * sizeof(float) : 0);
    static EnvSwitch wv("GAMER_GEMM_AS_WAVES");
    const int nw = d->sw_hm ? 4 : (wv.is_set() ? (wv.get(4) == 8 ? 8 : 4) : ((b_kc && d->groups == 1 && d->N >= 512 && AS_WAVES == 4) ? 8 : AS_WAVES));
    const dim3 grid((d->M + 32 * nw - 1) / (32 * nw) + (p.group_offsets ? d->groups : 0));
#define GAMER_LAUNCH_AS_W(KPV, WRCV, EPIV, NWV)                                                                               \
    do {                                                                                                                      \
        static bool attr_dev[MAX_DEVICES] = {};                                                                               \
        if (!attr_dev[current_device()]) {                                                                                    \
            const hipError_t e = hipFuncSetAttribute(reinterpret_cast<const void*>(gemm_as_kernel<KPV, WRCV, EPIV, NWV>),     \
                                                     hipFuncAttributeMaxDynamicSharedMemorySize, (int)shmem);                 \
            if (e != hipSuccess) { set_error("gamer_gemm_f32_split: hipFuncSetAttribute failed: %s", hipGetErrorString(e)); return (int)e; } \
            attr_dev[current_device()] = true;                                                                                \
        }                                                                                                                     \
        hipLaunchKernelGGL((gemm_as_kernel<KPV, WRCV, EPIV, NWV>), grid, dim3(64 * NWV), shmem, st, p);                        \
    } while (0)
#define GAMER_LAUNCH_AS(KPV, WRCV, EPIV)                                                                                      \
    do { if (nw == 8) GAMER_LAUNCH_AS_W(KPV, WRCV, EPIV, 8); else GAMER_LAUNCH_AS_W(KPV, WRCV, EPIV, 4); } while (0)
    if (b_kc && d->sw_hm) {
        switch (kp) {
            case 1: GAMER_LAUNCH_AS_W(1, false, 5, 4); break;
            case 2: GAMER_LAUNCH_AS_W(2, false, 5, 4); break;
            case 3: GAMER_LAUNCH_AS_W(3, false, 5, 4); break;
            default: GAMER_LAUNCH_AS_W(4, false, 5, 4); break;
        }
    } else if (b_kc) {
        switch (kp) {
            case 1: GAMER_LAUNCH_AS(1, false, 0); break;
            case 2: GAMER_LAUNCH_AS(2, false, 0); break;
            case 3: GAMER_LAUNCH_AS(3, false, 0); break;
            default: GAMER_LAUNCH_AS(4, false, 0); break;
        }
    } else if (d->sw_gu) {
        GAMER_LAUNCH_AS(4, true, 4);
    } else if (d->rowdot_out) {
        GAMER_LAUNCH_AS(4, true, 2);
    } else {
        GAMER_LAUNCH_AS(4, true, 0);
    }
#undef GAMER_LAUNCH_AS
#undef GAMER_LAUNCH_AS_W
    GAMER_CHECK_LAUNCH("gamer_gemm_f32_split/activation-stationary");
    g_as_launches.fetch_add(1, std::memory_order_relaxed);
    return 0;
}

}

extern "C" long long gamer_debug_gemm_as_launches(void) { return gamer::g_as_launches.load(std::memory_order_relaxed); }
```

### gamer_amd/engine.py

```python
from __future__ import annotations

import contextlib
import functools
import math
import os
from types import SimpleNamespace
from typing import Dict, List, Optional, Tuple

import torch

from . import ops
from .config import Qwen3MultiConfig

IGNORE_INDEX = -100


def _round_up(x: int, m: int) -> int:
    return (x + m - 1) // m * m


class _FlatLayout:

    def __init__(self, decay: List[Tuple[str, tuple]], nodecay: List[Tuple[str, tuple]]):
        self.entries: Dict[str, Tuple[int, tuple]] = {}
# ... 256 lines not shown
            self.dqkv = buf("dqkv", (T, QKV), act)
            self.dq = buf("dq", (T, NQ), act)
            self.dk = buf("dk", (T, NKV), act)
            self.dao = buf("dao", (T, NQ), act)
            self.delta = buf("delta", (B, nq, S), f32)
            n_norm = (3 if crosses else 2) * L + 1 + (1 if injects else 0)
            self.norm_partial = buf("norm_partial", (n_norm, 2048, H), f32)
            self.qk_partial = buf("qk_partial", (ops.qknorm_partial_numel(cfg.num_behavior + 1 if crosses else 0),), f32)
            self.ds_work = (buf("ds_work", (ops.attn_ds_work_numel(B, S, nq),), f32)
                            if (os.environ.get("GAMER_ATTN_SPILL", "1") != "0" and act == torch.float32 and self.spill)
                            else None)
        return self


def _matmul_arg(dtype: str, matmul: Optional[str]) -> str:
    if matmul is None:
        matmul = "split3" if dtype == "f32" else "f32"
    if matmul not in ops.MATMUL_MODES:
        raise ValueError(f"unknown matmul {matmul!r} ({sorted(ops.MATMUL_MODES)})")
    return matmul


def _check_split_dtype(dtype: str, matmul: str):
    if dtype != "f32" and matmul != "f32":
        raise ValueError("matmul='split3'/'split6'/'split9' is a form of the fp32 path; dtype='bf16' has its own GEMM")


def _check_dtype(dtype: str):
    if dtype not in ("f32", "bf16"):
        raise ValueError(f"unknown dtype {dtype!r} (f32 or bf16; the reference's --fp16 is not built)")


class Engine:

    N_NORM_PARTIAL = 512
    N_SUMSQ_PARTIAL = 1024

    def __new__(cls, *args, **kwargs):
        variant = kwargs.get("variant", args[3] if len(args) > 3 else "multi")
        if cls is Engine and variant in ("qwen3", "qwen3_session"):
            from .engine_qwen3 import Qwen3Engine, Qwen3SessionEngine
            cls = Qwen3Engine if variant == "qwen3" else Qwen3SessionEngine
        elif cls is Engine and variant == "qwen3moe":
            from .engine_qwen3moe import Qwen3MoeEngine
            cls = Qwen3MoeEngine
        return super().__new__(cls)

    def __init__(self, cfg: Qwen3MultiConfig, device="cuda", temperature: float = 1.0, variant: str = "multi",
                 dtype: str = "f32", matmul: Optional[str] = None, share_buffers_of: Optional["Engine"] = None,
                 deterministic: Optional[bool] = None):
        cfg.validate()
        matmul = _matmul_arg(dtype, matmul)
        _check_split_dtype(dtype, matmul)
        if variant not in self._VARIANTS:
            raise ValueError(f"unknown variant {variant!r} (multi, session, qwen3, qwen3_session or qwen3moe)")
        _check_dtype(dtype)
        self.key_spans = variant == "session"
        self._init_core(cfg, device, temperature, variant, dtype, matmul, share_buffers_of, deterministic)
        if self._amax is not None and self._amax.planes is not None and cfg.hidden_size == 256 and \
                os.environ.get("GAMER_GEMM_OSF", "0") == "1":
            self._amax.planes_t = torch.zeros(_round_up(self.layout.numel, 4), dtype=torch.float32, device=self.device)
        self.lut = cfg.behavior_lut().to(self.device)
        nb1 = cfg.num_behavior + 1
        self.split_inject = bool(self.dtype != "bf16" and os.environ.get("GAMER_SPLIT_INJECT", "1") != "0" and
                                 cfg.behavior_injection_decoder and cfg.num_experts * nb1 <= 64 and nb1 <= 16 and
                                 cfg.behavior_embedding_dim % 4 == 0 and cfg.behavior_embedding_dim <= 256 and cfg.shipped_ffn)
        self.position_table = (torch.tensor([0] + cfg.position_experts(), dtype=torch.int32, device=self.device)
                               if cfg.Moe_behavior_only else None)

    _VARIANTS = ("multi", "session")
    _item_aligned = True

    key_spans = False

    _layout_cls = ParamLayout
    _layer_cls = _LayerW
    _layer_t_cls = _LayerWT

    def _init_core(self, cfg, device, temperature, variant, dtype, matmul, share_buffers_of, deterministic):
        self.matmul, self.variant, self.dtype = matmul, variant, dtype
        self.deterministic = (os.environ.get("GAMER_DETERMINISTIC", "0") == "1") if deterministic is None else bool(deterministic)
        self.fuse_qkv = False
        self.fuse_qkv_bf16 = os.environ.get("GAMER_FUSE_QKV_BF16", "0") == "1"
        self.split_attention = True
        self.act_dtype = torch.float32 if dtype == "f32" else torch.bfloat16
        if not torch.cuda.is_available():
            raise RuntimeError("gamer_amd.Engine needs a HIP device (there is no CPU fallback)")
        from . import _lib
        _lib.load()
        self.cfg = cfg
        self.device = torch.device(device)
        self.temperature = float(temperature)
        self.layout = self._layout_cls(cfg)
        n = self.layout.numel
        if share_buffers_of is not None:
            if share_buffers_of.layout.numel != n or share_buffers_of.device != self.device:
                raise ValueError("share_buffers_of: the other engine has another parameter layout or device")
            self.flat_p, self.flat_g = share_buffers_of.flat_p, share_buffers_of.flat_g
        else:
            self.flat_p = torch.zeros(n, dtype=torch.float32, device=self.device)
            self.flat_g = torch.zeros(n, dtype=torch.float32, device=self.device)
        self.flat_m: Optional[torch.Tensor] = None
        self.flat_v: Optional[torch.Tensor] = None
        self.params = self.layout.views(self.flat_p)
        self.grads = self.layout.views(self.flat_g)
        L = cfg.num_hidden_layers
        self.W = [self._layer_cls(cfg, self.layout, self.flat_p, l) for l in range(L)]
        self.G = [self._layer_cls(cfg, self.layout, self.flat_g, l) for l in range(L)]
        self.shadow: Optional[Bf16Shadow] = None
        self.Wm, self.WT = self.W, None
        if dtype == "bf16":
            self.shadow = Bf16Shadow(cfg, self.layout, self.flat_p)
            self.Wm = [self._layer_cls(cfg, self.layout, self.shadow.flat16, l) for l in range(L)]
            self.WT = [self._layer_t_cls(cfg, self.shadow, l) for l in range(L)]
        self.weight_planes: Optional[torch.Tensor] = None
        if dtype == "f32" and matmul != "f32" and os.environ.get("GAMER_SPLIT_PLANES", "0") == "1":
            self.weight_planes = torch.zeros(3, _round_up(n, 4), dtype=torch.bfloat16, device=self.device)
        self.h2_attention = os.environ.get("GAMER_H2_ATTENTION", "1") != "0"
        self.gemm_c_amax = os.environ.get("GAMER_GEMM_CAMAX", "1") != "0"
        self._amax = None
        if dtype == "f32" and matmul == "split3":
            self._amax = ops.amax_reuse()
            self._amax.stable_range(self.flat_p.data_ptr(), self.flat_p.numel() * 4)
            if os.environ.get("GAMER_SPLIT3_PLANES", "1") != "0":
                self._amax.planes = torch.zeros(_round_up(n, 4), dtype=torch.float32, device=self.device)
        self._rope: Dict[int, Tuple[torch.Tensor, torch.Tensor]] = {}
        self._ws: Dict[bool, _Workspace] = {}
        self.ws: Optional[_Workspace] = None
        self.opt_step = 0
        self.dropout_step = 0
        self.base_seed = 0x5EED
        self.sumsq_partial = torch.empty(self.N_SUMSQ_PARTIAL, dtype=torch.float32, device=self.device)
        self.grad_norm = torch.zeros(1, dtype=torch.float32, device=self.device)
        self._norm_out_table = None
        self.fuse_swiglu_bwd = os.environ.get("GAMER_FUSE_SWIGLU_BWD", "1") != "0"
        self.ordered_embedding_grad = os.environ.get("GAMER_EMBEDDING_ATOMICS", "0") == "0"
        self._check_deterministic_embedding()
        self._saved = None

    def _check_deterministic_embedding(self):
        V = self.cfg.vocab_size
        if self.ordered_embedding_grad and V > 8191 and self.deterministic:
            raise RuntimeError(f"Engine(deterministic=True): the ordered embedding gradient takes at most 8191 vocabulary rows (V = {V}); "
                               "the float-atomics scatter it would fall back to is not reproducible")

    def init_weights(self, seed: int = 0):
        g = torch.Generator(device="cpu").manual_seed(seed)
        std = self.cfg.initializer_range
        for name, (off, shp) in self.layout.entries.items():
            n = math.prod(shp)
            if len(shp) == 1:
                self.flat_p[off:off + n].fill_(1.0)
            else:
                self.flat_p[off:off + n].copy_(torch.randn(n, generator=g) * std)
        self.params["model.embed_tokens.weight"][self.cfg.pad_token_id].zero_()

    def load_state_dict(self, sd: Dict[str, torch.Tensor]):
        missing = [k for k in self.layout.entries if k not in sd]
        if missing:
            raise KeyError(f"missing parameters: {missing[:5]}{'...' if len(missing) > 5 else ''}")
        for k, p in self.params.items():
            if tuple(sd[k].shape) != tuple(p.shape):
                raise ValueError(f"{k}: shape {tuple(sd[k].shape)} != {tuple(p.shape)}")
            p.copy_(sd[k].to(torch.float32))

    def rope(self, S: int):
# ... 39 lines not shown

    def _planes(self):
        wp = self.weight_planes
        return None if wp is None else (self.flat_p.data_ptr(), self.flat_p.numel() * 4, wp.data_ptr(), wp.stride(0))

    @ops.scoped_f32_matmul(lambda self, *a: self.matmul, lambda self, *a: self._planes())
    @ops.scoped_amax(lambda self, *a: self._amax)
    def forward(self, input_ids, attention_mask=None, actions=None, labels=None, num_items_in_batch=None,
                train: bool = False, dropout: Optional[bool] = None, act_zero_col: Optional[int] = None,
                uniform_len: int = 0, kv_sink=None, kv_dest=None, session_ids=None, extended_session_ids=None,
                last_row_logits: bool = False, hidden_sink: Optional[list] = None, rope_from_mask: bool = False):
        cfg = self.cfg
        B, S = input_ids.shape
        if train and self._item_aligned and S % cfg.num_positions != 0:
            raise ValueError(f"sequence length {S} is not a multiple of num_positions={cfg.num_positions} "
                             "(the router assumes item-aligned sequences, router.py:78-81)")
        if train and (act_zero_col is not None or uniform_len not in (0, S) or rope_from_mask):
            raise ValueError("act_zero_col / uniform_len / rope_from_mask are evaluation-only options")
        c = self._prologue(input_ids, attention_mask, labels, train, dropout, cfg.dropout_rate, kv_dest, hidden_sink,
                           last_row_logits, uniform_len,
                           eval_only="last_row_logits is an evaluation-only option" if last_row_logits else None,
                           f32_only=("generation (cached decode / re-run scoring) is built for dtype='f32' only"
                                     if last_row_logits or uniform_len not in (0, S) else None))
        ws, ids, am, bf16 = c.ws, c.ids, c.am, c.bf16
        T, H, nq, nkv, I, E = c.T, c.H, c.nq, c.nkv, c.I, cfg.num_experts
        NQ, NKV, QKV, eps, scale, cos, sin, p_res = c.NQ, c.NKV, c.QKV, c.eps, c.scale, c.cos, c.sin, c.p_res
        r = ws.router
        r["bad_token"].zero_()
        pos_ids = self._route(c, actions, act_zero_col, rope_from_mask)
        NB1 = cfg.num_behavior + 1
        if self.split_inject:
            ws.grp_key = ws._buf("grp_key", (B, S), torch.int32)
            ws.grp_offsets = ws._buf("grp_offsets", (E * NB1 + 1,), torch.int32)
            ws.row_group = ws._buf("row_group", (T,), torch.int32)
            torch.add(r["beh_idx"], r["expert"], alpha=NB1, out=ws.grp_key)
            ops.expert_lists(ws.grp_key, E * NB1, ws.perm, ws.slot, ws.grp_offsets, ws._buf("grp_work", ((B + 1) * E * NB1,), torch.int32))
            ws.offsets.copy_(ws.grp_offsets[::NB1])
            torch.index_select(ws.grp_key.view(-1), 0, ws.perm, out=ws.row_group)
            if self._amax is not None:
                self._amax.register(*[self.W[l].gu for l in cfg.behavior_injection_decoder])
        else:
            ops.expert_lists(r["expert"], E, ws.perm, ws.slot, ws.offsets, ws.work)
        if self._amax is not None and self._amax.planes_t is not None:
            for Wl in self.W:
                self._amax.register_transposed(Wl.self_attn["o"], 1, H, NQ)
                self._amax.register_transposed(Wl.down, Wl.ne, H, I)
                if Wl.cross:
                    self._amax.register_transposed(Wl.cross_attn["o"], 1, H, NQ)
        span_self = span_cross = None
        if self.variant == "session":
            if session_ids is None:
                raise ValueError("Session IDs must be provided to generate session-wise causal mask.")
            sid = session_ids.to(self.device, torch.int64).contiguous()
            ext = (extended_session_ids.to(self.device, torch.int64).contiguous()
                   if extended_session_ids is not None else None)
            if ws.session is None:
                i32 = torch.int32
                if "s_violations" not in ws._store:
                    ws._store["s_violations"] = torch.zeros(1, dtype=i32, device=self.device)
                ws.session = {"span_self": ws._buf("s_span_self", (B, S, 4), i32),
                              "span_cross": ws._buf("s_span_cross", (B, S, 4), i32),
                              "pos_ids": ws._buf("s_pos_ids", (B, S), i32), "violations": ws._store["s_violations"]}
            ws.session["violations"].zero_()
            ops.session_spans(sid, ext, am, cfg.num_positions, S, r, ws.session)
            span_self, span_cross, pos_ids = (ws.session["span_self"], ws.session["span_cross"],
                                              ws.session["pos_ids"])
        if cfg.cross_attention_decoder:
            ops.attn_row_order(r["empty_cross"], *ws.cross_order)
        ops.embedding_fwd(ids, self.params["model.embed_tokens.weight"], ws.x[0][0])

        fuse_qkv = ((self.fuse_qkv_bf16 if bf16 else self.fuse_qkv) and ops.qkv_fused_ok(ws.layers[0]["h1"], T, QKV)
                    and cfg.head_dim == 64)
        attention = functools.partial(self._attention, c)

        for l in range(cfg.num_hidden_layers):
            W, A, xs = self.W[l], ws.layers[l], ws.x[l]
            Wm = self.Wm[l]
            if hidden_sink is not None:
                hidden_sink.append(xs[0].view(B, S, H).clone())
            self._self_attention(c, l, r, span_self, pos_ids, fuse_qkv, kv_dest, kv_sink)
            xcur = xs[1]
            if W.cross:
                C, Cm = W.cross_attn, Wm.cross_attn
                ops.rmsnorm_fwd(xs[1], W.ln2, eps, A["h2"])
                qkv_x, k_x = kv_dest(l, "cross") if kv_dest is not None else (A["qkv_c"], A["k_c"])
                h2_hold = self._amax.hold(A["h2"]) if (self._amax is not None and not train) else None
                if h2_hold is not None:
                    h2_hold.__enter__()
                if fuse_qkv:
                    ops.gemm(A["h2"], H, 1, Cm["qkv"], H, 1, qkv_x, QKV, T, QKV, H,
                             qknorm=dict(wq=C["qn"], wk=C["kn"], eps=eps, cos=cos, sin=sin, q_rot=A["q_c"], k_rot=k_x,
                                         bias_q=C["bq"], bias_k=C["bk"], bias_v=C["bv"], act_idx=r["act_idx"],
                                         pos_ids=pos_ids, S=S, nq=nq, nkv=nkv))
                else:
                    ops.linear_fwd(A["h2"], H, Cm["qkv"], H, qkv_x, QKV, T, QKV, H)
                    ops.qknorm_rope_fwd(qkv_x, S, nq, nkv, C["qn"], C["kn"], eps, cos, sin, A["q_c"], k_x,
                                        bias_q=C["bq"], bias_k=C["bk"], bias_v=C["bv"], act_idx=r["act_idx"],
                                        pos_ids=pos_ids)
                if kv_sink is not None:
                    kv_sink(l, "cross", k_x, qkv_x[:, NQ + NKV:])
                if (last_row_logits and l == cfg.num_hidden_layers - 1 and span_cross is None and not bf16 and
                        os.environ.get("GAMER_PREFILL_LAST_ROW", "1") != "0"):
                    rows = torch.arange(B, device=self.device) * S + (S - 1)
                    f32 = dict(dtype=torch.float32, device=self.device)
                    q_l = A["q_c"].index_select(0, rows).contiguous()
                    key_ok = (r["kl_cross"].view(B, S) < r["ql_cross"].view(B, S)[:, S - 1:S]).to(torch.int32).contiguous()
                    uni = (r["empty_cross"].view(B, S)[:, S - 1] != 0).to(torch.int32).contiguous()
                    kg0 = torch.zeros(B, 1, NKV, **f32)
                    ao_l = torch.empty(B, NQ, **f32)
                    ops.attn_decode(q_l, k_x, qkv_x[:, NQ + NKV:], key_ok, kg0, kg0, 0, False, uni, B, 1, S, nq, nkv, scale, ao_l)
                    op_l, gate_l, x_cross_last = torch.empty(B, H, **f32), torch.empty(B, H, **f32), torch.empty(B, H, **f32)
                    ops.linear_fwd(ao_l, NQ, Cm["o"], NQ, op_l, H, B, H, NQ)
                    ops.linear_fwd(A["h2"].index_select(0, rows).contiguous(), H, Cm["gate"], H, gate_l, H, B, H, H)
                    ops.silu_gate_fwd(op_l, gate_l, x_cross_last, resid=xs[1].index_select(0, rows).contiguous())
                    xcur = None
                else:
                    x_cross_last = None
                    attention(A["q_c"], k_x, qkv_x[:, NQ + NKV:], r["kl_cross"], r["ql_cross"], r["empty_cross"],
                              r["tile_empty_cross"], self._seed(l, 2), A["ao_c"], A["lse_c"], ws.cross_order, span_cross)
                if x_cross_last is None:
                    ops.linear_fwd(A["ao_c"], NQ, Cm["o"], NQ, A["op_c"], H, T, H, NQ)
                    ops.linear_fwd(A["h2"], H, Cm["gate"], H, A["gate_c"], H, T, H, H)
                if h2_hold is not None:
                    h2_hold.__exit__(None, None, None)
                if x_cross_last is None:
                    ops.silu_gate_fwd(A["op_c"], A["gate_c"], xs[2], resid=xs[1], p=p_res, seed=self._seed(l, 3))
                    xcur = xs[2]
            din = W.din
            if last_row_logits and l == cfg.num_hidden_layers - 1:
                rows = torch.arange(B, device=self.device) * S + (S - 1)
                xl = x_cross_last if (W.cross and x_cross_last is not None) else xcur.index_select(0, rows).contiguous()
                f32 = dict(dtype=torch.float32, device=self.device)
                beh = r["beh_idx"].view(-1).index_select(0, rows).contiguous() if W.inject else None
                x_last = torch.empty(B, H, **f32)
                self.ffn_rows(W, (S - 1) % cfg.num_positions, xl, beh, x_last)
                break
            xnext = ws.x[l + 1][0] if l + 1 < cfg.num_hidden_layers else ws.x_final
            if not self._shipped_ffn_layer(W):
                self._ffn_fwd_plain(c, l, xcur, xnext)
                continue
            grp = dict(groups=E, group_offsets=ws.offsets)
            if W.inject and self.split_inject:
                hin = A["hin"].view(-1)[:T * H].view(T, H)
                ops.rmsnorm_fwd(xcur, W.ln3, eps, hin, H, ws.slot)
                tb = ws._buf((f"l{l}_" if train else "l_") + "inject_tbl", (E * NB1, 2 * I))
                ops.inject_table_fwd(W.beh, W.gu, din, H, E, 2 * I, tb)
                if c.fuse_swiglu_fwd:
                    ops.gemm(hin, H, 1, Wm.gu, din, 1, A["gu"], 2 * I, T, 2 * I, H, strideB=2 * I * din, groups=E * NB1,
                             group_offsets=ws.grp_offsets, group_div=NB1, p_drop=p_res, seed=self._seed(l, 4),
                             swiglu_fwd=(A["hm"], tb, ws.row_group))
                else:
                    ops.linear_fwd(hin, H, Wm.gu, din, A["gu"], 2 * I, T, 2 * I, H, strideB=2 * I * din, **grp)
                    ops.swiglu_fwd_ld_tbl(A["gu"], 2 * I, T, I, p_res, self._seed(l, 4), A["hm"], tb, ws.row_group)
            else:
                ops.rmsnorm_fwd(xcur, W.ln3, eps, A["hin"], din, ws.slot)
                if W.inject:
                    ops.rowtable_fwd(W.beh, r["beh_idx"], A["hin"], din, H, ws.slot)
                if c.fuse_swiglu_fwd and din == H:
                    ops.gemm(A["hin"], din, 1, Wm.gu, din, 1, A["gu"], 2 * I, T, 2 * I, din, strideB=2 * I * din, p_drop=p_res,
                             seed=self._seed(l, 4), swiglu_fwd=(A["hm"], None, None), **grp)
                else:
                    ops.linear_fwd(A["hin"], din, Wm.gu, din, A["gu"], 2 * I, T, 2 * I, din, strideB=2 * I * din, **grp)
                    ops.swiglu_fwd_ld(A["gu"], 2 * I, T, I, p_res, self._seed(l, 4), A["hm"])
            ops.gemm(A["hm"], I, 1, Wm.down, I, 1, xnext, H, T, H, I, strideB=H * I, resid=xcur, row_map=ws.perm,
                     p_drop=p_res, seed=self._seed(l, 5), **grp)
        return self._head(c, x_last if last_row_logits else None, num_items_in_batch, hidden_sink)

    def _route(self, c, actions, act_zero_col, rope_from_mask: bool):
        if rope_from_mask:
            raise ValueError("rope_from_mask is an option of the models without behaviour levels")
        cfg, r, S = self.cfg, c.ws.router, c.S
        act = actions.to(self.device, torch.int64).contiguous() if actions is not None else None
        ops.router_fwd(c.ids, c.am, act, self.lut, cfg.num_positions, cfg.pad_token_id, cfg.eos_token_id, r)
        if self.position_table is not None:
            ops.router_position_table(r["expert"], self.position_table)
        if act_zero_col is None and S % cfg.num_positions == 1:
            act_zero_col = S - 1
        if act_zero_col is not None:
            r["act_idx"][:, act_zero_col] = 0
        return None

    def _shipped_ffn_layer(self, W) -> bool:
        return W.sparse and W.gated and not self.cfg.Moe_behavior_only

    def _ffn_rows(self, l: int):
        return self.ws.slot if self.W[l].sparse else None

    def _ffn_fwd_plain(self, c, l: int, xcur, xnext):
        ws, W, Wm, A = c.ws, self.W[l], self.Wm[l], c.ws.layers[l]
        T, H, I, din, nI = c.T, c.H, c.I, W.din, W.nI
        slot = ws.slot if W.sparse else None
        grp = dict(groups=W.ne, group_offsets=ws.offsets) if W.sparse else {}
        phantom = W.sparse and self.cfg.Moe_behavior_only
        ops.rmsnorm_fwd(xcur, W.ln3, c.eps, A["hin"], din, slot)
        if W.inject:
            ops.rowtable_fwd(W.beh, ws.router["beh_idx"], A["hin"], din, H, slot)
        gu = A["gu"].view(-1)[:T * nI].view(T, nI)
        if phantom:
            gu.zero_()
        ops.linear_fwd(A["hin"], din, Wm.gu, din, gu, nI, T, nI, din, **(dict(strideB=nI * din) if W.sparse else {}), **grp)
        if W.gated:
            ops.swiglu_fwd_ld(gu, nI, T, I, c.p_res, self._seed(l, 4), A["hm"])
        else:
            ops.silu_fwd_ld(gu, nI, T, I, c.p_res, self._seed(l, 4), A["hm"])
        if phantom:
            xnext.copy_(xcur)
        ops.gemm(A["hm"], I, 1, Wm.down, I, 1, xnext, H, T, H, I, resid=xcur, p_drop=c.p_res, seed=self._seed(l, 5),
                 **(dict(strideB=H * I, row_map=ws.perm) if W.sparse else {}), **grp)

    def _ffn_bwd_plain(self, c, l: int, xlast):
        ws, W, G, A = c.ws, self.W[l], self.G[l], c.ws.layers[l]
        WT = self.WT[l] if c.bf16 else None
        T, H, I, din, nI = c.T, c.H, c.I, W.din, W.nI
        t0 = ws.tmpH[0]
        slot = ws.slot if W.sparse else None
        grp = dict(groups=W.ne, group_offsets=ws.offsets) if W.sparse else {}
        sB = (lambda n: dict(strideB=n)) if W.sparse else (lambda n: {})
        sC = (lambda n: dict(strideC=n)) if W.sparse else (lambda n: {})
        if W.sparse and self.cfg.Moe_behavior_only:
            ws.dhm.zero_()
            ws.dhin.zero_()
        with c.hold(t0):
            ops.linear_wgrad(t0, H, A["hm"], I, G.down, I, T, H, I, **sC(H * I), **grp)
            self._dgrad(c, t0, H, W.down, WT.down if c.bf16 else None, I, ws.dhm, I, H, I, **sB(H * I), **grp)
        gu = A["gu"].view(-1)[:T * nI].view(T, nI)
        if W.gated:
            ops.swiglu_bwd_ld(gu, nI, T, I, ws.dhm, c.p_res, self._seed(l, 4))
        else:
            ops.silu_bwd_ld(gu, nI, T, I, ws.dhm, c.p_res, self._seed(l, 4))
        with c.hold(gu):
            ops.linear_wgrad(gu, nI, A["hin"], din, G.gu, din, T, nI, din, **sC(nI * din), **grp)
            self._dgrad(c, gu, nI, W.gu, WT.gu if c.bf16 else None, din, ws.dhin, din, nI, din, **sB(nI * din), **grp)
        if W.inject:
            ops.rowtable_bwd(ws.dhin, din, H, ws.router["beh_idx"], G.beh, slot, partial=ws.norm_partial[-1])
        self._norm_bwd(c, xlast, W.ln3, ws.dhin, din, G.ln3, True, slot,
                       branch=None if W.cross else (self._seed(l, 1), None))

    def ffn_rows(self, W, pos: int, x, beh, out):
        cfg = self.cfg
        B, H, I, din, nI = x.shape[0], cfg.hidden_size, cfg.intermediate_size, W.din, W.nI
        e = cfg.position_experts()[pos] if W.sparse else 0
        if e >= W.ne:
            out.copy_(x)
            return
        f32 = dict(dtype=torch.float32, device=self.device)
        hin = torch.empty(B, din, **f32)
        ops.rmsnorm_fwd(x, W.ln3, float(cfg.rms_norm_eps), hin, din)
        if W.inject:
            ops.rowtable_fwd(W.beh, beh, hin, din, H)
        gu, hm = torch.empty(B, nI, **f32), torch.empty(B, I, **f32)
        ops.linear_fwd(hin, din, W.gu[e * nI:(e + 1) * nI], din, gu, nI, B, nI, din)
        if W.gated:
            ops.swiglu_fwd_ld(gu, nI, B, I, 0.0, 0, hm)
        else:
            ops.silu_fwd_ld(gu, nI, B, I, 0.0, 0, hm)
        ops.gemm(hm, I, 1, W.down[e * H:(e + 1) * H], I, 1, out, H, B, H, I, resid=x)

    def _pass(self, B: int, S: int, p_res: float, p_att: float) -> SimpleNamespace:
        cfg = self.cfg
        c = SimpleNamespace(B=B, S=S, T=B * S, H=cfg.hidden_size, nq=cfg.num_attention_heads, nkv=cfg.num_key_value_heads,
                            dh=cfg.head_dim, I=cfg.intermediate_size, eps=float(cfg.rms_norm_eps), p_res=p_res, p_att=p_att,
                            bf16=self.dtype == "bf16")
        c.NQ, c.NKV = c.nq * c.dh, c.nkv * c.dh
        c.QKV = c.NQ + 2 * c.NKV
        c.scale = float(c.dh) ** -0.5
        c.cos, c.sin = self.rope(S)
        c.split_attn = self.split_attention and self.matmul != "f32" and not c.bf16
        c.h2 = c.split_attn and self.h2_attention and self.matmul == "split3" and p_att < 0.75
        c.fuse_swiglu_fwd = not c.bf16 and self.matmul == "split3" and os.environ.get("GAMER_FUSE_SWIGLU_FWD", "1") != "0"
        c.fuse_swiglu_bwd = (c.bf16 or self.matmul == "split3") and self.fuse_swiglu_bwd
        return c

    def _prologue(self, input_ids, attention_mask, labels, train, dropout, dropout_rate, kv_dest, hidden_sink,
                  last_row_logits, uniform_len, eval_only: Optional[str], f32_only: Optional[str]) -> SimpleNamespace:
        B, S = input_ids.shape
        if kv_dest is not None and train:
            raise ValueError("kv_dest is an evaluation-only option (the backward reads the workspace's q|k|v and keys)")
        if eval_only and (train or labels is not None):
            raise ValueError(eval_only)
        if hidden_sink is not None and last_row_logits:
            raise ValueError("hidden_sink needs the full-sequence forward")
        if self.dtype == "bf16":
            if f32_only:
                raise NotImplementedError(f32_only)
            self.shadow.refresh()
        if self.weight_planes is not None:
            ops.split3_planes(self.flat_p, self.weight_planes)
        use_drop = train if dropout is None else dropout
        c = self._pass(B, S, float(dropout_rate) if use_drop else 0.0,
                       float(self.cfg.attention_dropout) if use_drop else 0.0)
        if use_drop:
            self.dropout_step += 1
        ws = c.ws = self.ws = self.workspace(B, S, train)
        if self._amax is not None:
            self._amax.reset()
            if train:
                self._amax.stable(ws.xn, *[A[k] for A in ws.layers for k in ("h1", "h2", "ao", "ao_c", "hin", "hm") if k in A])
                if self.h2_attention:
                    self._amax.stable(*[A[k] for A in ws.layers for k in ("q", "k", "q_c", "k_c") if k in A],
                                      *[A[k][:, c.NQ + c.NKV:] for A in ws.layers for k in ("qkv", "qkv_c") if k in A])
        c.ids = input_ids.to(self.device, torch.int64).contiguous()
        c.am = attention_mask.to(self.device, torch.int64).contiguous() if attention_mask is not None else None
        c.lab = labels.to(self.device, torch.int64).contiguous() if labels is not None else None
        c.uniform_len, c.train = uniform_len, train
        if c.lab is not None:
            ws.bad_label.zero_()
            ops.check_labels(c.lab, self.cfg.vocab_size, IGNORE_INDEX, ws.bad_label)
        return c

    def _attention(self, c, qb, kb, vb, kl_, ql_, empty_, tile_empty_, seed_, ob, lseb, order_, span_):
        B, S, nq, nkv, NQ, NKV, QKV = c.B, c.S, c.nq, c.nkv, c.NQ, c.NKV, c.QKV
        if c.split_attn and (span_ is None or c.h2):
            ops.attn_fwd_split(qb, NQ, kb, NKV, vb, QKV, kl_, ql_, empty_, B, S, nq, nkv, c.scale, c.p_att, seed_, ob, lseb,
                               order=order_, h2=c.h2, uniform_len=c.uniform_len, q_span=span_)
        elif c.bf16:
            ord16 = (order_[0], order_[2], empty_) if (order_ is not None and span_ is None) else None
            ops.attn_fwd_bf16(qb, NQ, kb, NKV, vb, QKV, kl_, ql_, B, S, nq, nkv, c.scale, c.p_att, seed_, ob, lseb,
                              q_span=span_, order=ord16)
        else:
            ops.attn_fwd(qb, NQ, kb, NKV, vb, QKV, kl_, ql_, empty_, tile_empty_, B, S, nq, nkv, c.scale, c.p_att, seed_,
                         ob, lseb, order=order_, uniform_len=c.uniform_len, q_span=span_)

    def _self_attention(self, c, l: int, masks: dict, span, pos_ids, fuse_qkv: bool, kv_dest, kv_sink):
        W, Wm, A, xs = self.W[l], self.Wm[l], c.ws.layers[l], c.ws.x[l]
        T, H, NQ, NKV, QKV, eps = c.T, c.H, c.NQ, c.NKV, c.QKV, c.eps
        ops.rmsnorm_fwd(xs[0], W.ln1, eps, A["h1"])
        qkv_s, k_s = kv_dest(l, "self") if kv_dest is not None else (A["qkv"], A["k"])
        if fuse_qkv:
            ops.gemm(A["h1"], H, 1, Wm.self_attn["qkv"], H, 1, qkv_s, QKV, T, QKV, H,
                     qknorm=dict(wq=W.self_attn["qn"], wk=W.self_attn["kn"], eps=eps, cos=c.cos, sin=c.sin, q_rot=A["q"],
                                 k_rot=k_s, pos_ids=pos_ids, S=c.S, nq=c.nq, nkv=c.nkv))
        else:
            v_amax = dict(c_amax=(qkv_s[:, NQ + NKV:], NQ + NKV)) if (c.h2 and self.gemm_c_amax) else {}
            ops.linear_fwd(A["h1"], H, Wm.self_attn["qkv"], H, qkv_s, QKV, T, QKV, H, **v_amax)
            ops.qknorm_rope_fwd(qkv_s, c.S, c.nq, c.nkv, W.self_attn["qn"], W.self_attn["kn"], eps, c.cos, c.sin, A["q"], k_s,
                                pos_ids=pos_ids)
        if kv_sink is not None:
            kv_sink(l, "self", k_s, qkv_s[:, NQ + NKV:])
        self._attention(c, A["q"], k_s, qkv_s[:, NQ + NKV:], masks["kl_self"], None, masks["empty_self"],
                        masks["tile_empty_self"], self._seed(l, 0), A["ao"], A["lse"], None, span)
        ops.gemm(A["ao"], NQ, 1, Wm.self_attn["o"], NQ, 1, xs[1], H, T, H, NQ, resid=xs[0], p_drop=c.p_res,
                 seed=self._seed(l, 1))

    def _head(self, c, x_last: Optional[torch.Tensor], num_items_in_batch, hidden_sink):
        ws, B, S, H, eps = c.ws, c.B, c.S, c.H, c.eps
        V = self.cfg.vocab_size
        if x_last is not None:
            xn = torch.empty_like(x_last)
            ops.rmsnorm_fwd(x_last, self.params["model.norm.weight"], eps, xn)
            small = torch.empty(B, ws.ldl, dtype=torch.float32, device=self.device)
            ops.linear_fwd(xn, H, self.params["model.embed_tokens.weight"], H, small, ws.ldl, B, V, H)
            self._saved = None
            self.last_logits_buf = small
            return None, small.view(B, 1, ws.ldl)[:, :, :V]
        ops.rmsnorm_fwd(ws.x_final, self.params["model.norm.weight"], eps, ws.xn)
        if hidden_sink is not None:
            hidden_sink.append(ws.xn.view(B, S, H).clone())
        emb_m = self.shadow.params16["model.embed_tokens.weight"] if c.bf16 else self.params["model.embed_tokens.weight"]
        lab = c.lab
        head_alpha = (1.0 / self.temperature) if (lab is not None and ws.logits.dtype == torch.float32) else 1.0
        ops.linear_fwd(ws.xn, H, emb_m, H, ws.logits, ws.ldl, c.T, V, H, alpha=head_alpha)
        loss = None
        if lab is not None:
            ops.ce_fwd(ws.logits, ws.ldl, lab, V, 1.0 if head_alpha != 1.0 else self.temperature, IGNORE_INDEX, ws.lse_ce,
                       ws.row_loss, ws.loss_sum, ws.count)
            if torch.is_tensor(num_items_in_batch):
                num_items_in_batch = num_items_in_batch.to(self.device, torch.float32).reshape(1)
                loss = ws.loss_sum[0] / num_items_in_batch[0]
            elif num_items_in_batch is not None:
                loss = ws.loss_sum[0] / float(num_items_in_batch)
            else:
                loss = ws.loss_sum[0] / ws.count[0]
        self._saved = dict(ids=c.ids, labels=lab, num_items=num_items_in_batch, train=c.train, p_res=c.p_res, p_att=c.p_att,
                           B=B, S=S, dropout_step=self.dropout_step)
        return loss, ws.logits.view(B, S, ws.ldl)[:, :, :V]

    def check_inputs(self):
        n = int(self.ws.router["bad_token"].item())
        if n:
            raise IndexError(f"{n} item(s) start with a token that is not in config.behavior_maps "
                             "(the reference fails with an embedding IndexError, router.py:170-171)")
        n = int(self.ws.bad_label.item())
        if n:
            raise IndexError(f"{n} label(s) outside [0, vocab_size={self.cfg.vocab_size}) that are not -100 "
                             "(nn.CrossEntropyLoss raises 'Target out of bounds' in the reference)")
        if self.variant == "session" and self.ws.session is not None:
            n = int(self.ws.session["violations"].item())
            if n:
                raise ValueError(f"{n} row(s) with session ids that decrease along the sequence or RoPE positions "
                                 "outside [0, S): the session masks are built as causal key spans "
                                 "(gamer_session_spans), which needs the dataset's layout (SMB_dataset.py:194-222)")

    def zero_grad(self):
        ops.fill(self.flat_g, 0.0)

    @ops.scoped_f32_matmul(lambda self, *a: self.matmul, lambda self, *a: self._planes())
    @ops.scoped_amax(lambda self, *a: self._amax)
    def backward(self, dloss: float = 1.0, layer_done=None, dloss_dev: Optional[torch.Tensor] = None):
        sv = self._saved
        if sv is None or not sv["train"] or sv["labels"] is None:
            raise RuntimeError("backward() needs forward(train=True, labels=...) first")
        with ops.deterministic(True if self.deterministic else ops.DETERMINISTIC_WGRAD, bf16=True if self.deterministic else None):
            return self._backward(dloss, layer_done, dloss_dev)

    def _backward(self, dloss: float = 1.0, layer_done=None, dloss_dev: Optional[torch.Tensor] = None):
        cfg = self.cfg
        c = self._backward_head(dloss, dloss_dev, rows=self._ffn_rows(cfg.num_hidden_layers - 1))
        ws, B, S, T, H, I, E = c.ws, c.B, c.S, c.T, c.H, c.I, cfg.num_experts
        nq, nkv, NQ, NKV, QKV, eps, cos, sin, p_res = c.nq, c.nkv, c.NQ, c.NKV, c.QKV, c.eps, c.cos, c.sin, c.p_res
        NB1 = cfg.num_behavior + 1
        span_self = span_cross = pos_ids = None
        if self.variant == "session":
            span_self, span_cross, pos_ids = ws.session["span_self"], ws.session["span_cross"], ws.session["pos_ids"]
        r = ws.router
        NP = ws.norm_partial[-1]
        hold, fuse_delta, do_amax, fuse_swiglu_bwd = c.hold, c.fuse_delta, c.do_amax, c.fuse_swiglu_bwd
        dgrad, norm_bwd = functools.partial(self._dgrad, c), functools.partial(self._norm_bwd, c)
        attention_bwd = functools.partial(self._attention_bwd, c)
        t0, t1, t2, t3 = ws.tmpH
        bf16 = c.bf16
        for l in reversed(range(cfg.num_hidden_layers)):
            W, G, A, xs = self.W[l], self.G[l], ws.layers[l], ws.x[l]
            WT = self.WT[l] if bf16 else None
            din = W.din
            grp = dict(groups=E, group_offsets=ws.offsets)
            xlast = xs[2] if W.cross else xs[1]
            if not self._shipped_ffn_layer(W):
                self._ffn_bwd_plain(c, l, xlast)
            else:
                split_inj = W.inject and self.split_inject
                tb = ws._buf(f"l{l}_inject_tbl", (E * NB1, 2 * I)) if split_inj else None
                with hold(t0):
                    ops.linear_wgrad(t0, H, A["hm"], I, G.down, I, T, H, I, strideC=H * I, **grp)
                    if fuse_swiglu_bwd and split_inj:
                        ops.gemm(t0, H, 1, W.down, 1, I, ws.dhm, I, T, I, H, strideB=H * I, p_drop=p_res, seed=self._seed(l, 4),
                                 swiglu_bwd=(A["gu"], 2 * I), groups=E * NB1, group_offsets=ws.grp_offsets, group_div=NB1, sw_tbl=tb)
                    elif fuse_swiglu_bwd:
                        if bf16:
                            ops.linear_dgrad_t(t0, H, WT.down, WT.down.shape[1], ws.dhm, I, T, H, I, strideB=H * I, p_drop=p_res,
                                               seed=self._seed(l, 4), swiglu_bwd=(A["gu"], 2 * I), **grp)
                        else:
                            ops.gemm(t0, H, 1, W.down, 1, I, ws.dhm, I, T, I, H, strideB=H * I, p_drop=p_res, seed=self._seed(l, 4),
                                     swiglu_bwd=(A["gu"], 2 * I), **grp)
                    else:
# ... 200 lines not shown
```

### gamer_amd/ops.py

```python
from __future__ import annotations

import ctypes as C
from typing import Optional

import os

import torch

from . import _lib
from ._lib import GemmBf16Desc, GemmDesc, call, ptr, stream_ptr


def _sfx(t: torch.Tensor) -> str:
    if t.dtype == torch.float32:
        return ""
    if t.dtype == torch.bfloat16:
        return "_bf16"
    raise RuntimeError(f"activations must be float32 or bfloat16, got {t.dtype}")


def _chk(t: torch.Tensor, dtype, name: str):
    if not t.is_cuda:
        raise RuntimeError(f"{name} must be on the HIP device (gamer_amd has no CPU path)")
    if t.dtype != dtype:
# ... 352 lines not shown
        i, j = divmod(self.used, 1024)
        if i == len(self.pools):
            self.pools.append(torch.zeros(1024 * AMAX_WORDS, dtype=torch.int32, device=device))
        self.used += 1
        return self.pools[i].data_ptr() + 4 * AMAX_WORDS * j

    def preset(self, x, geom, accumulate=False):
        key = self._key(x.data_ptr(), geom)
        if accumulate and key in self.pending:
            return self.pending[key]
        if accumulate == "only":
            return None
        self.slots.pop(key, None)
        ptr_ = self.pending[key] = self._new_slot(x.device)
        return ptr_

    def peek(self, x, geom):
        key = self._key(x.data_ptr(), geom)
        return self.pending.get(key) or self.slots.get(key)

    def slot(self, x, geom):
        p = x.data_ptr()
        key = self._key(p, geom)
        keep = self._cached(p)
        if key in self.pending:
            ptr_ = self.pending.pop(key)
            if keep:
                self.slots[key] = ptr_
            return ptr_
        if keep and key in self.slots:
            return self.slots[key]
        ptr_ = self._new_slot(x.device)
        call("gamer_absmax_f32", ptr(x), *geom, ptr_, stream_ptr())
        if keep:
            self.slots[key] = ptr_
            if (len(key) == 3 and self.stable_ranges and key[2] % 4 == 0 and
                    self.stable_ranges[0][0] <= p < self.stable_ranges[0][0] + self.stable_ranges[0][1] and
                    not any(p_ < p + 4 * key[2] and p < p_ + 4 * n_ for (p_, n_) in self._wkeys)):
                self._wkeys.append((p, key[2]))
                self._wdev = x.device
        return ptr_


def _drop_pending_on_failure(name):
    if _AMAX_REUSE is not None:
        _AMAX_REUSE.pending.clear()


_lib.FAILURE_HOOKS.append(_drop_pending_on_failure)

_AMAX_ATTN = os.environ.get("GAMER_AMAX_ATTN", "1") != "0"


def _arm_sink(*outs):
    if _AMAX_REUSE is None or F32_MATMUL_TERMS != 3 or outs[0][0].dtype != torch.float32:
        return
    slots = [_AMAX_REUSE.preset(t, g, acc) for t, g, acc in outs]
    if slots[0] is None:
        return
    if len(slots) > 2:
        call("gamer_amax_sink3", slots[0], slots[1], slots[2])
    else:
        call("gamer_amax_sink", slots[0], slots[1] if len(slots) > 1 else None)


def scoped_amax(get_cache):
    import functools

    def deco(fn):
        @functools.wraps(fn)
        def wrapper(*args, **kwargs):
            cache = get_cache(*args)
            if cache is None:
                return fn(*args, **kwargs)
            with cache:
                return fn(*args, **kwargs)
        return wrapper
    return deco


def absmax_slot(x, batch, stride, rows, cols, ld):
    if _AMAX_REUSE is not None:
        return _AMAX_REUSE.slot(x, (batch, stride, rows, cols, ld))
    key = (x.device.index, stream_ptr())
    ring = _AMAX_RING.get(key)
    if ring is None:
        ring = _AMAX_RING[key] = [torch.zeros(_AMAX_SLOTS * AMAX_WORDS, dtype=torch.int32, device=x.device), 0]
    if ring[1] == _AMAX_SLOTS:
        ring[0].zero_()
        ring[1] = 0
    slot = ring[0].data_ptr() + 4 * AMAX_WORDS * ring[1]
    ring[1] += 1
    call("gamer_absmax_f32", ptr(x), batch, stride, rows, cols, ld, slot, stream_ptr())
    return slot


def split3_planes(x, planes):
    call("gamer_split3_planes", ptr(x), ptr(planes), x.numel(), planes.stride(0), stream_ptr())


DETERMINISTIC_WGRAD = os.environ.get("GAMER_WGRAD_TWO_PASS", "1") != "0"
DETERMINISTIC_WGRAD_BF16 = os.environ.get("GAMER_WGRAD_TWO_PASS_BF16", "0") == "1"
_WGRAD_WS = {}


class deterministic:

    def __init__(self, on: bool = True, bf16=None):
        self.on, self.bf16 = bool(on), bf16

    def __enter__(self):
        global DETERMINISTIC_WGRAD, DETERMINISTIC_WGRAD_BF16
        self.prev, DETERMINISTIC_WGRAD = DETERMINISTIC_WGRAD, self.on
        self.prev16 = DETERMINISTIC_WGRAD_BF16
        if self.bf16 is not None:
            DETERMINISTIC_WGRAD_BF16 = bool(self.bf16)
        return self

    def __exit__(self, *exc):
        global DETERMINISTIC_WGRAD, DETERMINISTIC_WGRAD_BF16
        DETERMINISTIC_WGRAD, DETERMINISTIC_WGRAD_BF16 = self.prev, self.prev16
        return False


def _wgrad_workspace(device, floats: int) -> torch.Tensor:
    t = _WGRAD_WS.get(device)
    if t is None or t.numel() < floats:
        _WGRAD_WS[device] = None
        t = _WGRAD_WS[device] = torch.empty(int(floats), dtype=torch.float32, device=device)
    return t


class split3_guard:

    def __init__(self, on: bool):
        self.on = bool(on)

    def __enter__(self):
        self.prev = _lib.load().gamer_split3_guard(1 if self.on else 0)
        return self

    def __exit__(self, *exc):
        _lib.load().gamer_split3_guard(self.prev)
        return False


def set_f32_matmul(mode) -> int:
    global F32_MATMUL_TERMS
    prev = F32_MATMUL_TERMS
    terms = MATMUL_MODES[mode] if isinstance(mode, str) else int(mode)
    if terms not in (0, 3, 6, 9):
        raise ValueError(f"fp32 matmul mode {mode!r}: one of {sorted(MATMUL_MODES)}")
    F32_MATMUL_TERMS = terms
    return prev


def gemm(A, a_rs, a_ks, Bm, b_rs, b_ks, Cm, ldc, M, N, K, alpha=1.0, accumulate=False, groups=1, group_mode=0,
         group_offsets=None, strideB=0, strideC=0, kchunk=0, resid=None, row_map=None, p_drop=0.0, seed=0,
         rowdot=None, qknorm=None, c_amax=None, swiglu_bwd=None, group_div=0, sw_tbl=None, swiglu_fwd=None):
    if A.dtype == torch.bfloat16:
        if group_div > 1 or sw_tbl is not None or swiglu_fwd is not None:
            raise RuntimeError("group_div / sw_tbl / swiglu_fwd are options of the fp32 GEMM")
        return _gemm_bf16(A, a_rs, a_ks, Bm, b_rs, b_ks, Cm, ldc, M, N, K, alpha, accumulate, groups, group_mode,
                          group_offsets, strideB, strideC, kchunk, resid, row_map, p_drop, seed, rowdot, qknorm, swiglu_bwd)
    d = GemmDesc()
    d.A = ptr(A); d.a_rs = a_rs; d.a_ks = a_ks
    d.B = ptr(Bm); d.b_rs = b_rs; d.b_ks = b_ks
    d.C = ptr(Cm); d.ldc = ldc
    d.M = M; d.N = N; d.K = K
    d.alpha = alpha
    d.accumulate = 1 if accumulate else 0
    d.groups = groups
    d.group_mode = group_mode
    d.group_offsets = ptr(group_offsets)
    d.strideB = strideB; d.strideC = strideC
    d.kchunk = kchunk
    d.resid = ptr(resid)
    d.row_map = ptr(row_map)
    d.p_drop = p_drop
    d.seed = seed
    if rowdot is not None:
        d.rowdot_other, d.rowdot_out, d.rowdot_S = ptr(rowdot[0]), ptr(rowdot[1]), int(rowdot[2])
    if qknorm is not None:
        q = qknorm
        d.qk_wq, d.qk_wk, d.qk_eps = ptr(q["wq"]), ptr(q["wk"]), float(q["eps"])
        d.qk_cos, d.qk_sin = ptr(q["cos"]), ptr(q["sin"])
        d.qk_bias_q, d.qk_bias_k, d.qk_bias_v = ptr(q.get("bias_q")), ptr(q.get("bias_k")), ptr(q.get("bias_v"))
        d.qk_act_idx, d.qk_pos_ids = ptr(q.get("act_idx")), ptr(q.get("pos_ids"))
        d.qk_q_rot, d.qk_k_rot = ptr(q["q_rot"]), ptr(q["k_rot"])
        d.qk_S, d.qk_nq, d.qk_nkv = int(q["S"]), int(q["nq"]), int(q["nkv"])
    if (c_amax is not None and _AMAX_REUSE is not None and F32_MATMUL_TERMS == 3 and group_mode == 0 and not accumulate
            and resid is None and qknorm is None and c_amax[1] % 64 == 0):
        view, col0 = c_amax
        slot_c = _AMAX_REUSE.preset(view, (1, 0, M, N - col0, ldc))
        d.amax_c, d.amax_c_col0 = slot_c, int(col0)
    if swiglu_bwd is not None:
        gu, ld_gu = swiglu_bwd
        d.sw_gu, d.sw_ld = ptr(gu), int(ld_gu)
        d.sw_tbl = ptr(sw_tbl)
        if _AMAX_REUSE is not None and F32_MATMUL_TERMS == 3 and ld_gu == 2 * N:
            d.amax_c, d.amax_c_col0 = _AMAX_REUSE.preset(gu, (1, 0, 1, M * ld_gu, M * ld_gu)), 0
    d.group_div = int(group_div)
    if swiglu_fwd is not None:
        hm, tbl, row_group = swiglu_fwd
        d.sw_hm, d.sw_tbl, d.sw_row_group = ptr(hm), ptr(tbl), ptr(row_group)
        if _AMAX_REUSE is not None and F32_MATMUL_TERMS == 3:
            d.amax_c, d.amax_c_col0 = _AMAX_REUSE.preset(hm, (1, 0, 1, M * (N // 2), M * (N // 2))), 0
    if group_mode == 1 and DETERMINISTIC_WGRAD:
        n_chunks = (K + kchunk - 1) // kchunk + (groups if group_offsets is not None else 0)
        need = n_chunks * ((M + 127) // 128) * ((N + 127) // 128) * 16384
        ws = _wgrad_workspace(A.device, need)
        d.wgrad_ws, d.wgrad_ws_floats = ws.data_ptr(), ws.numel()
    if F32_MATMUL_TERMS == 3:
        ga = (M, K, a_rs) if a_ks == 1 else (K, M, a_ks)
        gb = (N, K, b_rs) if b_ks == 1 else (K, N, b_ks)
        nb = (groups // max(1, int(group_div))) if (group_mode == 0 and groups > 1) else 1
        d.amax_a = absmax_slot(A, 1, 0, *ga)
        geom_b = (nb, strideB if nb > 1 else 0) + gb
        c = _AMAX_REUSE
        parent = c.plane_parent(Bm.data_ptr(), geom_b) if (c is not None and c.planes is not None and group_mode == 0) else None
        if parent is not None:
            d.amax_b = parent
            d.b_planes = c.planes.data_ptr() + (Bm.data_ptr() - c.stable_ranges[0][0])
            call("gamer_gemm_f32_split", C.byref(d), 3, stream_ptr())
            return
        d.amax_b = absmax_slot(Bm, *geom_b)
        if c is not None and c.planes is not None and group_mode == 0 and c._key(Bm.data_ptr(), geom_b) in c._plane_keys:
            d.b_planes = c.planes.data_ptr() + (Bm.data_ptr() - c.stable_ranges[0][0])
            if a_ks == 1 and b_ks == 1 and c._key(Bm.data_ptr(), geom_b) in c._tplane_keys:
                d.b_planes_t = c.planes_t.data_ptr() + (Bm.data_ptr() - c.stable_ranges[0][0])
        call("gamer_gemm_f32_split", C.byref(d), 3, stream_ptr())
        return
    if F32_MATMUL_TERMS:
        if WEIGHT_PLANES is not None and group_mode == 0:
            base, nbytes, pl, stride = WEIGHT_PLANES
            off = Bm.data_ptr() - base
            if 0 <= off < nbytes:
                d.b_planes, d.b_plane_stride = pl + off // 2, stride
        call("gamer_gemm_f32_split", C.byref(d), F32_MATMUL_TERMS, stream_ptr())
    else:
        call("gamer_gemm_f32", C.byref(d), stream_ptr())


def _gemm_bf16(A, a_rs, a_ks, Bm, b_rs, b_ks, Cm, ldc, M, N, K, alpha, accumulate, groups, group_mode, group_offsets,
               strideB, strideC, kchunk, resid, row_map, p_drop, seed, rowdot, qknorm=None, swiglu_bwd=None):
    if Bm.dtype != torch.bfloat16 or alpha != 1.0:
        raise RuntimeError("gamer_gemm_bf16 takes two bf16 operands and alpha = 1")
    d = GemmBf16Desc()
    if group_mode == 0:
        if a_ks != 1 or b_ks != 1:
            raise RuntimeError("bf16 GEMM: both operands must be k-contiguous (dgrad runs on the transposed weight copy)")
        d.lda, d.ldb = a_rs, b_rs
        want = torch.float32 if resid is not None else torch.bfloat16
    else:
        if a_rs != 1 or b_rs != 1:
            raise RuntimeError("bf16 wgrad: both operands must be token-major")
        d.lda, d.ldb = a_ks, b_ks
        want = torch.float32
    if Cm.dtype != want:
        raise RuntimeError(f"bf16 GEMM: C must be {want}, got {Cm.dtype}")
    d.A, d.B, d.C, d.ldc = ptr(A), ptr(Bm), ptr(Cm), ldc
    d.M, d.N, d.K = M, N, K
    d.accumulate = 1 if accumulate else 0
    d.groups, d.group_mode, d.group_offsets = groups, group_mode, ptr(group_offsets)
    d.strideB, d.strideC, d.kchunk = strideB, strideC, kchunk
    d.resid, d.row_map, d.p_drop, d.seed = ptr(resid), ptr(row_map), p_drop, seed
    if rowdot is not None:
        d.rowdot_other, d.rowdot_out, d.rowdot_S = ptr(rowdot[0]), ptr(rowdot[1]), int(rowdot[2])
    if qknorm is not None:
        q = qknorm
        d.qk_wq, d.qk_wk, d.qk_eps = ptr(q["wq"]), ptr(q["wk"]), float(q["eps"])
        d.qk_cos, d.qk_sin = ptr(q["cos"]), ptr(q["sin"])
        d.qk_bias_q, d.qk_bias_k, d.qk_bias_v = ptr(q.get("bias_q")), ptr(q.get("bias_k")), ptr(q.get("bias_v"))
        d.qk_act_idx, d.qk_pos_ids = ptr(q.get("act_idx")), ptr(q.get("pos_ids"))
        d.qk_q_rot, d.qk_k_rot = ptr(q["q_rot"]), ptr(q["k_rot"])
        d.qk_S, d.qk_nq, d.qk_nkv = int(q["S"]), int(q["nq"]), int(q["nkv"])
    if swiglu_bwd is not None:
        d.sw_gu, d.sw_ld = ptr(swiglu_bwd[0]), int(swiglu_bwd[1])
    if group_mode == 1 and DETERMINISTIC_WGRAD_BF16:
        n_chunks = (K + kchunk - 1) // kchunk + (groups if group_offsets is not None else 0)
        need = n_chunks * ((M + 127) // 128) * ((N + 127) // 128) * 16384
        ws = _wgrad_workspace(A.device, need)
        d.wgrad_ws, d.wgrad_ws_floats = ws.data_ptr(), ws.numel()
    call("gamer_gemm_bf16", C.byref(d), stream_ptr())


def linear_dgrad_t(dy, lddy, WT, ldwt, dx, lddx, M, K_out, N_in, accumulate=False, **grp):
    gemm(dy, lddy, 1, WT, ldwt, 1, dx, lddx, M, N_in, K_out, accumulate=accumulate, **grp)


def qkv_fused_ok(x, M: int, N: int) -> bool:
    return x.dtype in (torch.float32, torch.bfloat16) and M % 128 == 0 and N % 128 == 0


def linear_fwd(x, ldx, W, ldw, y, ldy, M, N, K, accumulate=False, **grp):
    gemm(x, ldx, 1, W, ldw, 1, y, ldy, M, N, K, accumulate=accumulate, **grp)


def linear_dgrad(dy, lddy, W, ldw, dx, lddx, M, N_out, K_in, accumulate=False, **grp):
    gemm(dy, lddy, 1, W, 1, ldw, dx, lddx, M, K_in, N_out, accumulate=accumulate, **grp)
# ... 667 lines not shown
```

### include/gamer_hip.h

```cpp
#ifndef GAMER_HIP_H
#define GAMER_HIP_H

#include <stdint.h>

#ifdef __cplusplus
extern "C" {
#endif

#define GAMER_ABI_VERSION 9
#define GAMER_AMAX_WORDS 256

typedef uint16_t gamer_bf16;

int gamer_abi_version(void);
const char* gamer_last_error(void);
int gamer_reload_env(void);

int gamer_router_fwd(const int64_t* ids, const int64_t* attn_mask, const int64_t* actions,
                     const int32_t* behavior_lut, int vocab, int B, int S, int num_positions,
                     int pad_id, int eos_id,
                     int32_t* expert, int32_t* beh_idx, int32_t* act_idx,
                     int32_t* kl_self, int32_t* kl_cross, int32_t* ql_cross,
                     int32_t* empty_self, int32_t* empty_cross,
                     int32_t* tile_empty_self, int32_t* tile_empty_cross,
// ... 22 lines not shown
                          int32_t* next_pos, int32_t* bad_token, void* stream);

int gamer_expert_lists(const int32_t* expert, int B, int S, int num_experts,
                       int32_t* perm, int32_t* slot, int32_t* offsets, int32_t* work, void* stream);
int gamer_router_position_table(int32_t* expert, int64_t n, const int32_t* table, int n_table, void* stream);

int gamer_embedding_fwd(const int64_t* ids, const float* W, int V, int T, int H, float* x, void* stream);
int gamer_embedding_bwd(const int64_t* ids, const float* dx, int V, int T, int H, int pad_id, float* dW,
                        void* stream);
int64_t gamer_embedding_bwd_ordered_ws_bytes(int V, int T, int H);
int gamer_embedding_bwd_ordered(const int64_t* ids, const float* dx, int V, int T, int H, int pad_id, float* dW,
                                void* ws, int64_t ws_bytes, void* stream);

int gamer_rmsnorm_fwd(const float* x, const float* w, int T, int H, float eps,
                      const int32_t* dst_rows, float* y, int ldy, void* stream);
int gamer_rmsnorm_bwd(const float* x, const float* w, const float* dy, int lddy,
                      const int32_t* dy_rows, int T, int H, float eps, int accumulate_dx,
                      float* dx, float* dw_partial, int n_partial,
                      float* mask_out, const int32_t* mask_rows, float p_drop, uint64_t seed, void* stream);
int gamer_rmsnorm_fwd_bf16(const float* x, const float* w, int T, int H, float eps,
                           const int32_t* dst_rows, gamer_bf16* y, int ldy, void* stream);
int gamer_rmsnorm_bwd_bf16(const float* x, const float* w, const gamer_bf16* dy, int lddy,
                           const int32_t* dy_rows, int T, int H, float eps, int accumulate_dx,
                           float* dx, float* dw_partial, int n_partial,
                           gamer_bf16* mask_out, const int32_t* mask_rows, float p_drop, uint64_t seed, void* stream);
int gamer_colsum_reduce(const float* partial, int rows, int cols, int accumulate, float* out,
                        void* stream);
int gamer_colsum_reduce_batched(const float* partial, int64_t stride, int rows, int cols, int n, float* const* outs,
                                int accumulate, void* stream);

int gamer_rowtable_fwd(const float* table, const int32_t* idx, const int32_t* dst_rows, int T, int E,
                       float* y, int ldy, int col0, void* stream);
int gamer_rowtable_bwd(const float* dy, int lddy, int col0, const int32_t* idx,
                       const int32_t* dy_rows, int T, int E, int n_rows_table, float* dtable,
                       float* partial, int64_t partial_numel, void* stream);
int gamer_rowtable_fwd_bf16(const float* table, const int32_t* idx, const int32_t* dst_rows, int T, int E,
                            gamer_bf16* y, int ldy, int col0, void* stream);
int gamer_rowtable_bwd_bf16(const gamer_bf16* dy, int lddy, int col0, const int32_t* idx,
                            const int32_t* dy_rows, int T, int E, int n_rows_table, float* dtable,
                            float* partial, int64_t partial_numel, void* stream);

typedef struct {
    const float* A; int64_t a_rs, a_ks;
    const float* B; int64_t b_rs, b_ks;
    float* C; int64_t ldc;
    int M, N, K;
    float alpha;
    int accumulate;
    int groups;
    int group_mode;
    const int32_t* group_offsets;
    int64_t strideB, strideC;
    int kchunk;
    const float* resid;
    const int32_t* row_map;
    float p_drop;
    uint64_t seed;
    const float* rowdot_other;
    float* rowdot_out;
    int rowdot_S;
    const float* qk_wq; const float* qk_wk;
    float qk_eps;
    const float* qk_cos; const float* qk_sin;
    const float* qk_bias_q; const float* qk_bias_k; const float* qk_bias_v;
    const int32_t* qk_act_idx;
    const int32_t* qk_pos_ids;
    float* qk_q_rot; float* qk_k_rot;
    int qk_S, qk_nq, qk_nkv;
    const gamer_bf16* b_planes;
    int64_t b_plane_stride;
    const uint32_t* amax_a;
    const uint32_t* amax_b;
    uint32_t* amax_c;
    int amax_c_col0;
    float* wgrad_ws;
    int64_t wgrad_ws_floats;
    float* sw_gu;
    int64_t sw_ld;
    int group_div;
    const float* sw_tbl;
    const gamer_bf16* b_planes_t;
    float* sw_hm;
    const int32_t* sw_row_group;
} gamer_gemm_desc;

int gamer_gemm_f32(const gamer_gemm_desc* d, void* stream);
int gamer_split2h_transpose_multi(const gamer_bf16* planes, const int64_t* table, int n, gamer_bf16* planes_t, void* stream);

int gamer_gemm_f32_split(const gamer_gemm_desc* d, int terms, void* stream);
int gamer_split3_guard(int on);
int gamer_absmax_f32(const float* x, int batch, int64_t stride, int rows, int cols, int64_t ld, uint32_t* out, void* stream);
int gamer_absmax_multi_f32(const float* base, const int64_t* table, int n, uint32_t* out, void* stream);
int gamer_split2h_planes_multi(const float* base, const int64_t* table, int n, const uint32_t* slots, gamer_bf16* planes,
                               void* stream);
int gamer_amax_sink(uint32_t* out0, uint32_t* out1);
int gamer_amax_sink3(uint32_t* out0, uint32_t* out1, uint32_t* out2);
int gamer_attn_split_amax(const uint32_t* q, const uint32_t* k, const uint32_t* v, const uint32_t* d_o);
int gamer_split3_planes(const float* x, gamer_bf16* planes, int64_t n, int64_t plane_stride, void* stream);

typedef struct {
    const gamer_bf16* A; int64_t lda;
    const gamer_bf16* B; int64_t ldb;
    void* C; int64_t ldc;
    int M, N, K;
    int accumulate;
    int groups;
    int group_mode;
    const int32_t* group_offsets;
    int64_t strideB, strideC;
    int kchunk;
    const float* resid;
    const int32_t* row_map;
    float p_drop;
    uint64_t seed;
    const gamer_bf16* rowdot_other;
    float* rowdot_out;
    int rowdot_S;
    const float* qk_wq; const float* qk_wk; float qk_eps;
    const float* qk_cos; const float* qk_sin;
    const float* qk_bias_q; const float* qk_bias_k; const float* qk_bias_v;
    const int32_t* qk_act_idx; const int32_t* qk_pos_ids;
    gamer_bf16* qk_q_rot; gamer_bf16* qk_k_rot;
    int qk_S, qk_nq, qk_nkv;
    gamer_bf16* sw_gu;
    int64_t sw_ld;
    float* wgrad_ws;
    int64_t wgrad_ws_floats;
} gamer_gemm_bf16_desc;

int gamer_gemm_bf16(const gamer_gemm_bf16_desc* d, void* stream);

int gamer_cast_params_bf16(const float* flat, gamer_bf16* out, gamer_bf16* out_t, const int64_t* table,
                           int n_entries, int n_tiles, void* stream);

int gamer_qknorm_rope_fwd(float* qkv, int T, int S, int nq, int nkv,
                          const float* wq, const float* wk, float eps,
                          const float* cos_t, const float* sin_t,
                          const float* bias_q, const float* bias_k, const float* bias_v,
                          const int32_t* act_idx,
                          float* q_rot, float* k_rot, const int32_t* pos_ids, void* stream);
int gamer_qknorm_rope_bwd(const float* qkv, const float* dq_rot, const float* dk_rot,
                          int T, int S, int nq, int nkv,
                          const float* wq, const float* wk, float eps,
                          const float* cos_t, const float* sin_t,
                          const float* bias_q, const float* bias_k,
                          const int32_t* act_idx, int nb1,
                          float* dqkv, float* dwq, float* dwk,
                          float* dbias_q, float* dbias_k, float* dbias_v, const int32_t* pos_ids,
                          float* partial, int64_t partial_numel, void* stream);
int gamer_qknorm_rope_fwd_bf16(gamer_bf16* qkv, int T, int S, int nq, int nkv,
                               const float* wq, const float* wk, float eps,
                               const float* cos_t, const float* sin_t,
                               const float* bias_q, const float* bias_k, const float* bias_v,
                               const int32_t* act_idx,
                               gamer_bf16* q_rot, gamer_bf16* k_rot, const int32_t* pos_ids, void* stream);
int gamer_qknorm_rope_bwd_bf16(const gamer_bf16* qkv, const gamer_bf16* dq_rot, const gamer_bf16* dk_rot,
                               int T, int S, int nq, int nkv,
                               const float* wq, const float* wk, float eps,
                               const float* cos_t, const float* sin_t,
                               const float* bias_q, const float* bias_k,
                               const int32_t* act_idx, int nb1,
                               gamer_bf16* dqkv, float* dwq, float* dwk,
                               float* dbias_q, float* dbias_k, float* dbias_v, const int32_t* pos_ids,
                               float* partial, int64_t partial_numel, void* stream);

int gamer_attn_row_order(const int32_t* row_empty, int B, int S, int32_t* perm, int32_t* tile_kind,
// ... 183 lines not shown
```

Measured before the change: 5069.

## Fuse RMSNorm prologue into split-3 GEMM kernel for attention, FFN and head inputs

Adds a norm_w/norm_out prologue to the gemm descriptor so the gemm_as kernel computes RMSNorm on each A row in registers, writes the normalized row to norm_out, and publishes its absmax from inside the kernel. This removes the separate rmsnorm launch and the separate absmax pass over the normalized activations before the QKV, FFN and LM-head GEMMs. Shapes the fused kernel cannot take fall back to a gathered rmsnorm plus a plain GEMM. The fused path only applies for K=256 with k-contiguous weights, adds register pressure to the kernel prologue, and changes the floating-point summation order of the norm.

```diff
diff --git a/gamer_amd/_lib.py b/gamer_amd/_lib.py
--- a/gamer_amd/_lib.py
+++ b/gamer_amd/_lib.py
@@ -53,6 +53,8 @@
         ("sw_gu", c_void_p), ("sw_ld", c_int64),
         ("group_div", c_int), ("sw_tbl", c_void_p), ("b_planes_t", c_void_p),
         ("sw_hm", c_void_p), ("sw_row_group", c_void_p),
+        ("norm_w", c_void_p), ("norm_eps", c_float), ("norm_out", c_void_p), ("norm_ld", c_int64),
+        ("norm_src_rows", c_void_p), ("amax_norm", c_void_p),
     ]
 
 
diff --git a/gamer_amd/csrc/common.h b/gamer_amd/csrc/common.h
--- a/gamer_amd/csrc/common.h
+++ b/gamer_amd/csrc/common.h
@@ -267,6 +267,16 @@
     return s * (1.f + x * (1.f - s));
 }
 
+__device__ __forceinline__ float rms_chunk_ss(const float4 v) {
+#pragma clang fp contract(off)
+    return ((v.x * v.x + v.y * v.y) + v.z * v.z) + v.w * v.w;
+}
+__device__ __forceinline__ float rms_rstd(float ss, float inv_h, float eps) { return rsqrtf(__builtin_fmaf(ss, inv_h, eps)); }
+__device__ __forceinline__ float4 rms_apply(const float4 w, const float4 v, float rstd) {
+    return make_float4(w.x * (v.x * rstd), w.y * (v.y * rstd), w.z * (v.z * rstd), w.w * (v.w * rstd));
+}
+int rmsnorm_fwd_gather(const float* x, const float* w, int T, int H, float eps, const int32_t* src_rows, float* y, int ldy, void* stream);
+
 bool gemm_as_eligible(const gamer_gemm_desc* d, bool a_kc, bool b_kc, const uint16_t* b_planes);
 int launch_gemm_as(const gamer_gemm_desc* d, const uint16_t* b_planes, bool b_kc, hipStream_t st);
 bool gemm_os_eligible(const gamer_gemm_desc* d, bool a_kc, bool b_kc, const uint16_t* b_planes);
diff --git a/gamer_amd/csrc/elementwise.hip b/gamer_amd/csrc/elementwise.hip
--- a/gamer_amd/csrc/elementwise.hip
+++ b/gamer_amd/csrc/elementwise.hip
@@ -255,7 +255,8 @@
 template <typename TY, int RMS_MAXC>
 __global__ void __launch_bounds__(EW_THREADS)
 rmsnorm_fwd_kernel(const float4* __restrict__ x, const float4* __restrict__ w, int T, int H4, float inv_h,
-                   float eps, const int32_t* __restrict__ dst_rows, TY* __restrict__ y, int ldy, uint32_t* __restrict__ amax_out) {
+                   float eps, const int32_t* __restrict__ dst_rows, TY* __restrict__ y, int ldy, uint32_t* __restrict__ amax_out,
+                   const int32_t* __restrict__ src_rows = nullptr) {
     __shared__ uint32_t amax_lds[4];
     uint32_t am = 0;
     const int lane = threadIdx.x & 63;
@@ -270,25 +271,22 @@
     for (int t = wave; t < T; t += nwaves) {
         float4 v[RMS_MAXC];
         float ss = 0.f;
+        const int64_t tin = src_rows ? src_rows[t] : t;
 #pragma unroll
         for (int i = 0; i < RMS_MAXC; ++i) {
             const int c = lane + 64 * i;
-            v[i] = (c < H4) ? x[(int64_t)t * H4 + c] : make_float4(0.f, 0.f, 0.f, 0.f);
-            ss += v[i].x * v[i].x + v[i].y * v[i].y + v[i].z * v[i].z + v[i].w * v[i].w;
+            v[i] = (c < H4) ? x[tin * H4 + c] : make_float4(0.f, 0.f, 0.f, 0.f);
+            ss += rms_chunk_ss(v[i]);
         }
         ss = wave_sum(ss);
-        const float rstd = rsqrtf(ss * inv_h + eps);
+        const float rstd = rms_rstd(ss, inv_h, eps);
         const int64_t r = dst_rows ? dst_rows[t] : t;
         TY* yrow = y + r * ldy;
 #pragma unroll
         for (int i = 0; i < RMS_MAXC; ++i) {
             const int c = lane + 64 * i;
             if (c < H4) {
-                float4 o;
-                o.x = wv[i].x * (v[i].x * rstd);
-                o.y = wv[i].y * (v[i].y * rstd);
-                o.z = wv[i].z * (v[i].z * rstd);
-                o.w = wv[i].w * (v[i].w * rstd);
+                const float4 o = rms_apply(wv[i], v[i], rstd);
                 st4(yrow + 4 * c, o);
                 am = amax_f4(am, o);
             }
@@ -1821,7 +1819,7 @@
 
 template <typename TY>
 static int rmsnorm_fwd_impl(const char* name, const float* x, const float* w, int T, int H, float eps,
-                            const int32_t* dst_rows, TY* y, int ldy, void* stream) {
+                            const int32_t* dst_rows, TY* y, int ldy, void* stream, const int32_t* src_rows = nullptr) {
     GAMER_CHECK_ARG(x && w && y, "%s: null pointer", name);
     GAMER_CHECK_ARG(T > 0 && H > 0 && H % 4 == 0 && H <= 256 * RMS_MAXC_BIG && ldy >= H && ldy % 4 == 0,
                     "%s: bad shape T=%d H=%d ldy=%d (H%%4==0, H<=1024, ldy%%4==0)", name, T, H, ldy);
@@ -1829,16 +1827,20 @@
     const AmaxSink sink = take_amax_sink();
     if (H <= 256)
         hipLaunchKernelGGL((rmsnorm_fwd_kernel<TY, 1>), dim3(grid_for_waves(T)), dim3(EW_THREADS), 0, ST(stream),
-                           (const float4*)x, (const float4*)w, T, H / 4, 1.f / (float)H, eps, dst_rows, y, ldy, sink.out[0]);
+                           (const float4*)x, (const float4*)w, T, H / 4, 1.f / (float)H, eps, dst_rows, y, ldy, sink.out[0], src_rows);
     else
         hipLaunchKernelGGL((rmsnorm_fwd_kernel<TY, RMS_MAXC_BIG>), dim3(grid_for_waves(T)), dim3(EW_THREADS), 0, ST(stream),
-                           (const float4*)x, (const float4*)w, T, H / 4, 1.f / (float)H, eps, dst_rows, y, ldy, sink.out[0]);
+                           (const float4*)x, (const float4*)w, T, H / 4, 1.f / (float)H, eps, dst_rows, y, ldy, sink.out[0], src_rows);
     GAMER_CHECK_LAUNCH(name);
     return 0;
 }
 extern "C" int gamer_rmsnorm_fwd(const float* x, const float* w, int T, int H, float eps, const int32_t* dst_rows,
                                  float* y, int ldy, void* stream) {
     return rmsnorm_fwd_impl<float>("gamer_rmsnorm_fwd", x, w, T, H, eps, dst_rows, y, ldy, stream);
+}
+int gamer::rmsnorm_fwd_gather(const float* x, const float* w, int T, int H, float eps, const int32_t* src_rows, float* y, int ldy,
+                              void* stream) {
+    return rmsnorm_fwd_impl<float>("gamer_gemm_f32/rmsnorm", x, w, T, H, eps, nullptr, y, ldy, stream, src_rows);
 }
 extern "C" int gamer_rmsnorm_fwd_bf16(const float* x, const float* w, int T, int H, float eps, const int32_t* dst_rows,
                                       gamer_bf16* y, int ldy, void* stream) {
diff --git a/gamer_amd/csrc/gemm.hip b/gamer_amd/csrc/gemm.hip
--- a/gamer_amd/csrc/gemm.hip
+++ b/gamer_amd/csrc/gemm.hip
@@ -1401,7 +1401,21 @@
                                   aligned16(d->C) && (!d->sw_tbl || d->sw_row_group) && d->p_drop >= 0.f && d->p_drop < 1.f),
                     "gamer_gemm_f32: the SwiGLU-forward epilogue (sw_hm) needs a Linear-forward layout with N = 2 I (N=%d), alpha = 1, no other "
                     "epilogue, and sw_row_group with sw_tbl", d->N);
+    GAMER_CHECK_ARG(!d->norm_w || (d->group_mode == 0 && a_kc && d->a_rs == d->K && d->norm_out && d->norm_ld >= d->K && d->norm_ld % 4 == 0 &&
+                                   d->K % 4 == 0 && d->K <= 1024 && aligned16(d->norm_w) && aligned16(d->norm_out) &&
+                                   (split != 3 || !d->amax_norm || d->amax_a == d->amax_norm)),
+                    "gamer_gemm_f32: the RMSNorm prologue (norm_w) needs a dense k-contiguous A (a_rs = K = %d <= 1024), group_mode 0, norm_out "
+                    "with norm_ld >= K (norm_ld=%lld), 16-byte alignment, and amax_a = amax_norm in the terms = 3 form", d->K, (long long)d->norm_ld);
     if (split == 3 && gemm_as_eligible(d, a_kc, b_kc, p.b_planes)) return launch_gemm_as(d, p.b_planes, b_kc, (hipStream_t)stream);
+    if (d->norm_w) {
+        if (d->amax_norm) gamer_amax_sink(d->amax_norm, nullptr);
+        const int rcn = rmsnorm_fwd_gather(d->A, d->norm_w, d->M, d->K, d->norm_eps, d->norm_src_rows, d->norm_out, (int)d->norm_ld, stream);
+        if (rcn) return rcn;
+        gamer_gemm_desc d2 = *d;
+        d2.A = d->norm_out; d2.a_rs = d->norm_ld;
+        d2.norm_w = nullptr; d2.norm_out = nullptr; d2.norm_src_rows = nullptr; d2.amax_norm = nullptr;
+        return gemm_entry(&d2, stream, split);
+    }
     if (d->sw_hm) {
         gamer_gemm_desc d2 = *d;
         d2.sw_hm = nullptr; d2.sw_row_group = nullptr; d2.sw_tbl = nullptr; d2.amax_c = nullptr;
diff --git a/gamer_amd/csrc/gemm_as.hip b/gamer_amd/csrc/gemm_as.hip
--- a/gamer_amd/csrc/gemm_as.hip
+++ b/gamer_amd/csrc/gemm_as.hip
@@ -39,15 +39,18 @@
     const float* rowdot_other; float* rowdot_out; int rowdot_S;
     float* sw_gu; int64_t sw_ld; float p_drop; uint64_t seed;
     float* hm; const float* tbl; int group_div;
+    const float* norm_w; float norm_eps, norm_inv_h; float* norm_out; int64_t norm_ld; const int32_t* norm_src_rows; uint32_t* amax_norm;
 };
 
-template <int KP, bool WRC, int EPI, int NW>
+template <int KP, bool WRC, int EPI, int NW, bool NORM = false>
 __global__ void __launch_bounds__(64 * NW, AS_DEPTH == 2 ? 1 : 8 / NW)
 gemm_as_kernel(const AsParams p) {
+    static_assert(!NORM || (KP == 4 && !WRC), "the RMSNorm prologue is built for K = 256, W k-contiguous");
     constexpr int AS_WAVES_K = NW, AS_THREADS_K = 64 * NW;
     extern __shared__ __attribute__((aligned(16))) unsigned char as_raw[];
     bf16_t* const wimg = reinterpret_cast<bf16_t*>(as_raw);
     __shared__ uint32_t amax_word;
+    __shared__ uint32_t amax_norm_word;
     const int tid = threadIdx.x, lane = tid & 63, w = tid >> 6;
     const int r = lane & 31, h = lane >> 5;
     int row0 = blockIdx.x * (32 * AS_WAVES_K), row_end = p.M, grp = 0;
@@ -67,18 +70,43 @@
     }
     const int m = row0 + w * 32 + r;
     const bool valid_m = m < row_end;
-    if (tid == 0) amax_word = 0;
+    if (tid == 0) { amax_word = 0; if (NORM) amax_norm_word = 0; }
 
     bf16x8 af[2][KP * 4];
     float row_inv;
+    float nmax = 0.f;
     {
-        const float* arow = p.A + (int64_t)(valid_m ? m : row_end - 1) * p.lda + 8 * h;
+        int64_t arow_i = valid_m ? m : row_end - 1;
+        if (NORM && p.norm_src_rows) arow_i = p.norm_src_rows[arow_i];
+        const float* arow = p.A + arow_i * p.lda + 8 * h;
         float4 raw[KP * 8];
 #pragma unroll
         for (int s = 0; s < KP * 4; ++s) {
             raw[2 * s] = *reinterpret_cast<const float4*>(arow + 16 * s);
             raw[2 * s + 1] = *reinterpret_cast<const float4*>(arow + 16 * s + 4);
         }
+        if (NORM) {
+            if (!valid_m) {
+#pragma unroll
+                for (int i = 0; i < KP * 8; ++i) raw[i] = make_float4(0.f, 0.f, 0.f, 0.f);
+            }
+            auto t1 = [&](int s, int b) { return rms_chunk_ss(raw[2 * s + b]) + rms_chunk_ss(raw[2 * (s + 8) + b]); };
+            auto t2 = [&](int s, int b) { return t1(s, b) + t1(s + 4, b); };
+            auto t3 = [&](int s, int b) { return t2(s, b) + t2(s + 2, b); };
+            auto t4 = [&](int b) { return t3(0, b) + t3(1, b); };
+            const float ss = xor32_sum(t4(0)) + xor32_sum(t4(1));
+            const float rstd = rms_rstd(ss, p.norm_inv_h, p.norm_eps);
+            const float* wrow = p.norm_w + 8 * h;
+            float* yrow = p.norm_out + (int64_t)m * p.norm_ld + 8 * h;
+#pragma unroll
+            for (int s = 0; s < KP * 4; ++s)
+#pragma unroll
+                for (int j = 0; j < 2; ++j) {
+                    raw[2 * s + j] = rms_apply(*reinterpret_cast<const float4*>(wrow + 16 * s + 4 * j), raw[2 * s + j], rstd);
+                    if (valid_m) *reinterpret_cast<float4*>(yrow + 16 * s + 4 * j) = raw[2 * s + j];
+                }
+            __builtin_amdgcn_sched_barrier(0);
+        }
         float mx = 0.f;
 #pragma unroll
         for (int i = 0; i < KP * 8; ++i) {
@@ -86,6 +114,7 @@
             mx = fmaxf(fmaxf(fmaxf(mx, fabsf(raw[i].x)), fabsf(raw[i].y)), fmaxf(fabsf(raw[i].z), fabsf(raw[i].w)));
         }
         mx = xor32_max(mx);
+        if (NORM) nmax = mx;
         float s_row = 1.f;
         row_inv = 1.f;
         if (mx > 0.f) scale_from_amax(__float_as_uint(mx), s_row, row_inv);
@@ -317,13 +346,21 @@
             bufc = b2;
         }
     }
-    if (p.amax_c) {
+    const bool pub_norm = NORM && p.amax_norm != nullptr;
+    if (p.amax_c || pub_norm) {
         uint32_t mw = __float_as_uint((EPI == 4 || EPI == 5) ? emax : cmax);
 #pragma unroll
         for (int o2 = 32; o2 > 0; o2 >>= 1) mw = max(mw, (uint32_t)__shfl_xor((int)mw, o2, 64));
-        if (lane == 0 && mw) atomicMax(&amax_word, mw);
+        if (lane == 0 && mw && p.amax_c) atomicMax(&amax_word, mw);
+        if (pub_norm) {
+            uint32_t nw_ = __float_as_uint(nmax);
+#pragma unroll
+            for (int o2 = 16; o2 > 0; o2 >>= 1) nw_ = max(nw_, (uint32_t)__shfl_xor((int)nw_, o2, 64));
+            if (lane == 0 && nw_) atomicMax(&amax_norm_word, nw_);
+        }
         __syncthreads();
-        if (tid == 0 && amax_word) amax_publish(amax_word, p.amax_c, blockIdx.x);
+        if (tid == 0 && p.amax_c && amax_word) amax_publish(amax_word, p.amax_c, blockIdx.x);
+        if (tid == 0 && pub_norm && amax_norm_word) amax_publish(amax_norm_word, p.amax_norm, blockIdx.x);
     }
 }
 
@@ -350,6 +387,12 @@
     if (d->a_rs % 4 != 0 || d->ldc % 4 != 0 || !aligned16(d->C) || !aligned16(b_planes)) return false;
     if (d->groups != 1 && (!d->group_offsets || d->strideC != 0)) return false;
     if (d->groups == 1 && d->group_offsets) return false;
+    if (d->norm_w) {
+        static EnvSwitch swn("GAMER_GEMM_AS_NORM");
+        if (swn.get(1) == 0 || !b_kc || d->K != 256 || !d->norm_out || d->norm_ld < d->K || d->norm_ld % 4 != 0 || !aligned16(d->norm_out) ||
+            !aligned16(d->norm_w))
+            return false;
+    }
     if (b_kc) {
         if (d->accumulate || d->rowdot_out || d->sw_gu || d->b_rs % 4 != 0) return false;
         if (d->groups != 1 && d->amax_c && !d->sw_hm) return false;
@@ -383,25 +426,32 @@
     p.rowdot_other = d->rowdot_other; p.rowdot_out = d->rowdot_out; p.rowdot_S = d->rowdot_S;
     p.sw_gu = d->sw_gu; p.sw_ld = d->sw_ld; p.p_drop = d->p_drop; p.seed = d->seed;
     p.hm = d->sw_hm; p.tbl = d->sw_hm ? d->sw_tbl : nullptr; p.group_div = d->group_div > 1 ? d->group_div : 1;
+    p.norm_w = d->norm_w; p.norm_eps = d->norm_eps; p.norm_inv_h = 1.f / (float)d->K; p.norm_out = d->norm_out; p.norm_ld = d->norm_ld;
+    p.norm_src_rows = d->norm_src_rows; p.amax_norm = d->amax_norm;
     const int kp = d->K / 64;
     const size_t shmem = (size_t)(AS_DEPTH == 2 ? 3 : 2) * 2 * kp * AS_PANEL * sizeof(bf16_t) + (d->sw_hm ? (size_t)d->N * sizeof(float) : 0);
     static EnvSwitch wv("GAMER_GEMM_AS_WAVES");
     const int nw = d->sw_hm ? 4 : (wv.is_set() ? (wv.get(4) == 8 ? 8 : 4) : ((b_kc && d->groups == 1 && d->N >= 512 && AS_WAVES == 4) ? 8 : AS_WAVES));
     const dim3 grid((d->M + 32 * nw - 1) / (32 * nw) + (p.group_offsets ? d->groups : 0));
-#define GAMER_LAUNCH_AS_W(KPV, WRCV, EPIV, NWV)                                                                               \
+#define GAMER_LAUNCH_AS_WN(KPV, WRCV, EPIV, NWV, NORMV)                                                                        \
     do {                                                                                                                      \
-        static bool attr_dev[MAX_DEVICES] = {};                                                                               \
-        if (!attr_dev[current_device()]) {                                                                                    \
-            const hipError_t e = hipFuncSetAttribute(reinterpret_cast<const void*>(gemm_as_kernel<KPV, WRCV, EPIV, NWV>),     \
+        static std::atomic<size_t> attr_dev[MAX_DEVICES] = {};                                                                \
+        if (attr_dev[current_device()].load(std::memory_order_relaxed) < shmem) {                                             \
+            const hipError_t e = hipFuncSetAttribute(reinterpret_cast<const void*>(gemm_as_kernel<KPV, WRCV, EPIV, NWV, NORMV>), \
                                                      hipFuncAttributeMaxDynamicSharedMemorySize, (int)shmem);                 \
             if (e != hipSuccess) { set_error("gamer_gemm_f32_split: hipFuncSetAttribute failed: %s", hipGetErrorString(e)); return (int)e; } \
-            attr_dev[current_device()] = true;                                                                                \
+            attr_dev[current_device()].store(shmem, std::memory_order_relaxed);                                               \
         }                                                                                                                     \
-        hipLaunchKernelGGL((gemm_as_kernel<KPV, WRCV, EPIV, NWV>), grid, dim3(64 * NWV), shmem, st, p);                        \
+        hipLaunchKernelGGL((gemm_as_kernel<KPV, WRCV, EPIV, NWV, NORMV>), grid, dim3(64 * NWV), shmem, st, p);                 \
     } while (0)
+#define GAMER_LAUNCH_AS_W(KPV, WRCV, EPIV, NWV) GAMER_LAUNCH_AS_WN(KPV, WRCV, EPIV, NWV, false)
 #define GAMER_LAUNCH_AS(KPV, WRCV, EPIV)                                                                                      \
     do { if (nw == 8) GAMER_LAUNCH_AS_W(KPV, WRCV, EPIV, 8); else GAMER_LAUNCH_AS_W(KPV, WRCV, EPIV, 4); } while (0)
-    if (b_kc && d->sw_hm) {
+    if (d->norm_w) {
+        if (d->sw_hm) GAMER_LAUNCH_AS_WN(4, false, 5, 4, true);
+        else if (nw == 8) GAMER_LAUNCH_AS_WN(4, false, 0, 8, true);
+        else GAMER_LAUNCH_AS_WN(4, false, 0, 4, true);
+    } else if (b_kc && d->sw_hm) {
         switch (kp) {
             case 1: GAMER_LAUNCH_AS_W(1, false, 5, 4); break;
             case 2: GAMER_LAUNCH_AS_W(2, false, 5, 4); break;
@@ -424,6 +474,7 @@
     }
 #undef GAMER_LAUNCH_AS
 #undef GAMER_LAUNCH_AS_W
+#undef GAMER_LAUNCH_AS_WN
     GAMER_CHECK_LAUNCH("gamer_gemm_f32_split/activation-stationary");
     g_as_launches.fetch_add(1, std::memory_order_relaxed);
     return 0;
diff --git a/gamer_amd/engine.py b/gamer_amd/engine.py
--- a/gamer_amd/engine.py
+++ b/gamer_amd/engine.py
@@ -362,6 +362,7 @@
         self.deterministic = (os.environ.get("GAMER_DETERMINISTIC", "0") == "1") if deterministic is None else bool(deterministic)
         self.fuse_qkv = False
         self.fuse_qkv_bf16 = os.environ.get("GAMER_FUSE_QKV_BF16", "0") == "1"
+        self.gemm_as_norm = os.environ.get("GAMER_GEMM_AS_NORM", "0") == "1"
         self.split_attention = True
         self.act_dtype = torch.float32 if dtype == "f32" else torch.bfloat16
         if not torch.cuda.is_available():
@@ -567,18 +568,21 @@
             xcur = xs[1]
             if W.cross:
                 C, Cm = W.cross_attn, Wm.cross_attn
-                ops.rmsnorm_fwd(xs[1], W.ln2, eps, A["h2"])
+                norm2 = dict(w=W.ln2, eps=eps, out=A["h2"]) if self.gemm_as_norm else None
+                if norm2 is None:
+                    ops.rmsnorm_fwd(xs[1], W.ln2, eps, A["h2"])
+                x_in = xs[1] if norm2 is not None else A["h2"]
                 qkv_x, k_x = kv_dest(l, "cross") if kv_dest is not None else (A["qkv_c"], A["k_c"])
                 h2_hold = self._amax.hold(A["h2"]) if (self._amax is not None and not train) else None
                 if h2_hold is not None:
                     h2_hold.__enter__()
                 if fuse_qkv:
-                    ops.gemm(A["h2"], H, 1, Cm["qkv"], H, 1, qkv_x, QKV, T, QKV, H,
+                    ops.gemm(x_in, H, 1, Cm["qkv"], H, 1, qkv_x, QKV, T, QKV, H, norm=norm2,
                              qknorm=dict(wq=C["qn"], wk=C["kn"], eps=eps, cos=cos, sin=sin, q_rot=A["q_c"], k_rot=k_x,
                                          bias_q=C["bq"], bias_k=C["bk"], bias_v=C["bv"], act_idx=r["act_idx"],
                                          pos_ids=pos_ids, S=S, nq=nq, nkv=nkv))
                 else:
-                    ops.linear_fwd(A["h2"], H, Cm["qkv"], H, qkv_x, QKV, T, QKV, H)
+                    ops.linear_fwd(x_in, H, Cm["qkv"], H, qkv_x, QKV, T, QKV, H, norm=norm2)
                     ops.qknorm_rope_fwd(qkv_x, S, nq, nkv, C["qn"], C["kn"], eps, cos, sin, A["q_c"], k_x,
                                         bias_q=C["bq"], bias_k=C["bk"], bias_v=C["bv"], act_idx=r["act_idx"],
                                         pos_ids=pos_ids)
@@ -627,25 +631,33 @@
             grp = dict(groups=E, group_offsets=ws.offsets)
             if W.inject and self.split_inject:
                 hin = A["hin"].view(-1)[:T * H].view(T, H)
-                ops.rmsnorm_fwd(xcur, W.ln3, eps, hin, H, ws.slot)
+                norm3 = dict(w=W.ln3, eps=eps, out=hin, ld=H, src_rows=ws.perm, dst_rows=ws.slot) if self.gemm_as_norm else None
+                if norm3 is None:
+                    ops.rmsnorm_fwd(xcur, W.ln3, eps, hin, H, ws.slot)
+                x_in = xcur if norm3 is not None else hin
                 tb = ws._buf((f"l{l}_" if train else "l_") + "inject_tbl", (E * NB1, 2 * I))
                 ops.inject_table_fwd(W.beh, W.gu, din, H, E, 2 * I, tb)
                 if c.fuse_swiglu_fwd:
-                    ops.gemm(hin, H, 1, Wm.gu, din, 1, A["gu"], 2 * I, T, 2 * I, H, strideB=2 * I * din, groups=E * NB1,
+                    ops.gemm(x_in, H, 1, Wm.gu, din, 1, A["gu"], 2 * I, T, 2 * I, H, strideB=2 * I * din, groups=E * NB1,
                              group_offsets=ws.grp_offsets, group_div=NB1, p_drop=p_res, seed=self._seed(l, 4),
-                             swiglu_fwd=(A["hm"], tb, ws.row_group))
+                             swiglu_fwd=(A["hm"], tb, ws.row_group), norm=norm3)
                 else:
-                    ops.linear_fwd(hin, H, Wm.gu, din, A["gu"], 2 * I, T, 2 * I, H, strideB=2 * I * din, **grp)
+                    ops.linear_fwd(x_in, H, Wm.gu, din, A["gu"], 2 * I, T, 2 * I, H, strideB=2 * I * din, norm=norm3, **grp)
                     ops.swiglu_fwd_ld_tbl(A["gu"], 2 * I, T, I, p_res, self._seed(l, 4), A["hm"], tb, ws.row_group)
             else:
-                ops.rmsnorm_fwd(xcur, W.ln3, eps, A["hin"], din, ws.slot)
+                norm3 = (dict(w=W.ln3, eps=eps, out=A["hin"], ld=din, src_rows=ws.perm, dst_rows=ws.slot)
+                         if (din == H and self.gemm_as_norm) else None)
+                if norm3 is None:
+                    ops.rmsnorm_fwd(xcur, W.ln3, eps, A["hin"], din, ws.slot)
                 if W.inject:
                     ops.rowtable_fwd(W.beh, r["beh_idx"], A["hin"], din, H, ws.slot)
+                ffn_in = dict(norm=norm3) if norm3 is not None else {}
                 if c.fuse_swiglu_fwd and din == H:
-                    ops.gemm(A["hin"], din, 1, Wm.gu, din, 1, A["gu"], 2 * I, T, 2 * I, din, strideB=2 * I * din, p_drop=p_res,
-                             seed=self._seed(l, 4), swiglu_fwd=(A["hm"], None, None), **grp)
+                    ops.gemm(xcur, din, 1, Wm.gu, din, 1, A["gu"], 2 * I, T, 2 * I, din, strideB=2 * I * din, p_drop=p_res,
+                             seed=self._seed(l, 4), swiglu_fwd=(A["hm"], None, None), norm=norm3, **grp)
                 else:
-                    ops.linear_fwd(A["hin"], din, Wm.gu, din, A["gu"], 2 * I, T, 2 * I, din, strideB=2 * I * din, **grp)
+                    ops.linear_fwd(A["hin"] if norm3 is None else xcur, din, Wm.gu, din, A["gu"], 2 * I, T, 2 * I, din,
+                                   strideB=2 * I * din, **ffn_in, **grp)
                     ops.swiglu_fwd_ld(A["gu"], 2 * I, T, I, p_res, self._seed(l, 4), A["hm"])
             ops.gemm(A["hm"], I, 1, Wm.down, I, 1, xnext, H, T, H, I, strideB=H * I, resid=xcur, row_map=ws.perm,
                      p_drop=p_res, seed=self._seed(l, 5), **grp)
@@ -809,15 +821,18 @@
     def _self_attention(self, c, l: int, masks: dict, span, pos_ids, fuse_qkv: bool, kv_dest, kv_sink):
         W, Wm, A, xs = self.W[l], self.Wm[l], c.ws.layers[l], c.ws.x[l]
         T, H, NQ, NKV, QKV, eps = c.T, c.H, c.NQ, c.NKV, c.QKV, c.eps
-        ops.rmsnorm_fwd(xs[0], W.ln1, eps, A["h1"])
+        norm1 = dict(w=W.ln1, eps=eps, out=A["h1"]) if self.gemm_as_norm else None
+        if norm1 is None:
+            ops.rmsnorm_fwd(xs[0], W.ln1, eps, A["h1"])
+        x_in = xs[0] if norm1 is not None else A["h1"]
         qkv_s, k_s = kv_dest(l, "self") if kv_dest is not None else (A["qkv"], A["k"])
         if fuse_qkv:
-            ops.gemm(A["h1"], H, 1, Wm.self_attn["qkv"], H, 1, qkv_s, QKV, T, QKV, H,
+            ops.gemm(x_in, H, 1, Wm.self_attn["qkv"], H, 1, qkv_s, QKV, T, QKV, H, norm=norm1,
                      qknorm=dict(wq=W.self_attn["qn"], wk=W.self_attn["kn"], eps=eps, cos=c.cos, sin=c.sin, q_rot=A["q"],
                                  k_rot=k_s, pos_ids=pos_ids, S=c.S, nq=c.nq, nkv=c.nkv))
         else:
             v_amax = dict(c_amax=(qkv_s[:, NQ + NKV:], NQ + NKV)) if (c.h2 and self.gemm_c_amax) else {}
-            ops.linear_fwd(A["h1"], H, Wm.self_attn["qkv"], H, qkv_s, QKV, T, QKV, H, **v_amax)
+            ops.linear_fwd(x_in, H, Wm.self_attn["qkv"], H, qkv_s, QKV, T, QKV, H, norm=norm1, **v_amax)
             ops.qknorm_rope_fwd(qkv_s, c.S, c.nq, c.nkv, W.self_attn["qn"], W.self_attn["kn"], eps, c.cos, c.sin, A["q"], k_s,
                                 pos_ids=pos_ids)
         if kv_sink is not None:
@@ -838,13 +853,16 @@
             self._saved = None
             self.last_logits_buf = small
             return None, small.view(B, 1, ws.ldl)[:, :, :V]
-        ops.rmsnorm_fwd(ws.x_final, self.params["model.norm.weight"], eps, ws.xn)
-        if hidden_sink is not None:
-            hidden_sink.append(ws.xn.view(B, S, H).clone())
+        norm_f = dict(w=self.params["model.norm.weight"], eps=eps, out=ws.xn) if self.gemm_as_norm else None
+        if norm_f is None:
+            ops.rmsnorm_fwd(ws.x_final, self.params["model.norm.weight"], eps, ws.xn)
         emb_m = self.shadow.params16["model.embed_tokens.weight"] if c.bf16 else self.params["model.embed_tokens.weight"]
         lab = c.lab
         head_alpha = (1.0 / self.temperature) if (lab is not None and ws.logits.dtype == torch.float32) else 1.0
-        ops.linear_fwd(ws.xn, H, emb_m, H, ws.logits, ws.ldl, c.T, V, H, alpha=head_alpha)
+        ops.linear_fwd(ws.x_final if norm_f is not None else ws.xn, H, emb_m, H, ws.logits, ws.ldl, c.T, V, H, alpha=head_alpha,
+                       norm=norm_f)
+        if hidden_sink is not None:
+            hidden_sink.append(ws.xn.view(B, S, H).clone())
         loss = None
         if lab is not None:
             ops.ce_fwd(ws.logits, ws.ldl, lab, V, 1.0 if head_alpha != 1.0 else self.temperature, IGNORE_INDEX, ws.lse_ce,
diff --git a/gamer_amd/ops.py b/gamer_amd/ops.py
--- a/gamer_amd/ops.py
+++ b/gamer_amd/ops.py
@@ -458,16 +458,21 @@
 def absmax_slot(x, batch, stride, rows, cols, ld):
     if _AMAX_REUSE is not None:
         return _AMAX_REUSE.slot(x, (batch, stride, rows, cols, ld))
-    key = (x.device.index, stream_ptr())
+    slot = _fresh_slot(x.device)
+    call("gamer_absmax_f32", ptr(x), batch, stride, rows, cols, ld, slot, stream_ptr())
+    return slot
+
+
+def _fresh_slot(device):
+    key = (device.index, stream_ptr())
     ring = _AMAX_RING.get(key)
     if ring is None:
-        ring = _AMAX_RING[key] = [torch.zeros(_AMAX_SLOTS * AMAX_WORDS, dtype=torch.int32, device=x.device), 0]
+        ring = _AMAX_RING[key] = [torch.zeros(_AMAX_SLOTS * AMAX_WORDS, dtype=torch.int32, device=device), 0]
     if ring[1] == _AMAX_SLOTS:
         ring[0].zero_()
         ring[1] = 0
     slot = ring[0].data_ptr() + 4 * AMAX_WORDS * ring[1]
     ring[1] += 1
-    call("gamer_absmax_f32", ptr(x), batch, stride, rows, cols, ld, slot, stream_ptr())
     return slot
 
 
@@ -533,7 +538,12 @@
 
 def gemm(A, a_rs, a_ks, Bm, b_rs, b_ks, Cm, ldc, M, N, K, alpha=1.0, accumulate=False, groups=1, group_mode=0,
          group_offsets=None, strideB=0, strideC=0, kchunk=0, resid=None, row_map=None, p_drop=0.0, seed=0,
-         rowdot=None, qknorm=None, c_amax=None, swiglu_bwd=None, group_div=0, sw_tbl=None, swiglu_fwd=None):
+         rowdot=None, qknorm=None, c_amax=None, swiglu_bwd=None, group_div=0, sw_tbl=None, swiglu_fwd=None, norm=None):
+    if norm is not None and (norm["out"].dtype != torch.float32 or A.dtype != torch.float32):
+        if norm.get("src_rows") is not None and norm.get("dst_rows") is None:
+            raise RuntimeError("norm= with src_rows on bf16 activations needs dst_rows (the inverse row list)")
+        rmsnorm_fwd(A, norm["w"], norm["eps"], norm["out"], norm.get("ld"), norm.get("dst_rows"))
+        A, a_rs, norm = norm["out"], (norm.get("ld") or norm["out"].stride(0)), None
     if A.dtype == torch.bfloat16:
         if group_div > 1 or sw_tbl is not None or swiglu_fwd is not None:
             raise RuntimeError("group_div / sw_tbl / swiglu_fwd are options of the fp32 GEMM")
@@ -587,11 +597,25 @@
         need = n_chunks * ((M + 127) // 128) * ((N + 127) // 128) * 16384
         ws = _wgrad_workspace(A.device, need)
         d.wgrad_ws, d.wgrad_ws_floats = ws.data_ptr(), ws.numel()
+    if norm is not None:
+        if a_ks != 1 or a_rs != K or group_mode != 0:
+            raise RuntimeError("norm= needs a dense k-contiguous A (a_rs = K) and group_mode 0")
+        n_out = norm["out"]
+        n_ld = int(norm.get("ld") or n_out.stride(0))
+        d.norm_w, d.norm_eps, d.norm_out, d.norm_ld = ptr(norm["w"]), float(norm["eps"]), ptr(n_out), n_ld
+        d.norm_src_rows = ptr(norm.get("src_rows"))
     if F32_MATMUL_TERMS == 3:
         ga = (M, K, a_rs) if a_ks == 1 else (K, M, a_ks)
         gb = (N, K, b_rs) if b_ks == 1 else (K, N, b_ks)
         nb = (groups // max(1, int(group_div))) if (group_mode == 0 and groups > 1) else 1
-        d.amax_a = absmax_slot(A, 1, 0, *ga)
+        if norm is not None:
+            if _AMAX_REUSE is not None:
+                _AMAX_REUSE.preset(n_out, (1, 0, M, K, n_ld))
+                d.amax_a = d.amax_norm = _AMAX_REUSE.slot(n_out, (1, 0, M, K, n_ld))
+            else:
+                d.amax_a = d.amax_norm = _fresh_slot(n_out.device)
+        else:
+            d.amax_a = absmax_slot(A, 1, 0, *ga)
         geom_b = (nb, strideB if nb > 1 else 0) + gb
         c = _AMAX_REUSE
         parent = c.plane_parent(Bm.data_ptr(), geom_b) if (c is not None and c.planes is not None and group_mode == 0) else None
diff --git a/include/gamer_hip.h b/include/gamer_hip.h
--- a/include/gamer_hip.h
+++ b/include/gamer_hip.h
@@ -128,6 +128,12 @@
     const gamer_bf16* b_planes_t;
     float* sw_hm;
     const int32_t* sw_row_group;
+    const float* norm_w;
+    float norm_eps;
+    float* norm_out;
+    int64_t norm_ld;
+    const int32_t* norm_src_rows;
+    uint32_t* amax_norm;
 } gamer_gemm_desc;
 
 int gamer_gemm_f32(const gamer_gemm_desc* d, void* stream);
```

Result: no change. 5049 (-0.4%).
